# yardenas/ethz-safe-learning

Hardware: NVIDIA B200
Metric: CEM-MPC plans/sec (PointGoal1 shape; ensemble transitions/sec alongside) (higher is better)
Workload: dtype bf16

## Files before the change

### ethz-safe-learning_b200/csrc/rollout_tc.cu

```cuda
#include <cuda_bf16.h>

#include <cstdlib>
#include <type_traits>

#include "common.cuh"
#include "internal.h"
#include "rollout_params.cuh"
#include "tc_head.cuh"
#include "tc_ptx.cuh"

namespace simba {

#ifdef SIMBA_TC_TIMELINE
#define TL(ev)                                                                                   \
  do {                                                                                           \
    if (tl_who >= 0 && blockIdx.x == 0)                                                          \
      prm.timeline[(tl_who * 64 + tl_t) * 64 + (ev)] = clock64();  \
  } while (0)
#else
#define TL(ev) do { } while (0)
#endif

namespace {

constexpr int kU = 128;
constexpr int kMaxO = 60;
constexpr int kAtomBytes = 128 * 128;
constexpr int kBiasBlockBytes = 4096;
constexpr int kBoundThreads = 640;

__host__ __device__ constexpr uint32_t tc_weight_bytes(int L) { return kAtomBytes + (uint32_t)L * 2 * kAtomBytes; }
__host__ __device__ constexpr uint32_t tc_member_bytes(int L) {
  return tc_weight_bytes(L) + (uint32_t)(L + 1) * kBiasBlockBytes;
}
__host__ __device__ constexpr bool tc_l0_pad_bias(int in_dim) { return in_dim + 2 <= 64; }

struct TileInfo {
  int32_t member, k0, count, valid;
};

template <int NB, int kThreads>
struct NoiseSmem {
  uint4* base;
  __device__ __forceinline__ uint4 get4(int b) const { return base[b * kThreads]; }
  __device__ __forceinline__ void put4(int b, uint4 v) { base[b * kThreads] = v; }
  __device__ __forceinline__ void put4_dyn(int b, uint4 v) { base[b * kThreads] = v; }
};
template <int NB>
struct NoiseRegs {
  uint4 v[NB];
  __device__ __forceinline__ uint4 get4(int b) const { return v[b]; }
  __device__ __forceinline__ void put4(int b, uint4 x) { v[b] = x; }
  __device__ __forceinline__ void put4_dyn(int b, uint4 x) {
#pragma unroll
    for (int i = 0; i < NB; ++i)
      if (i == b) v[i] = x;
  }
};

struct AStoreTmem {
  uint32_t t_a;
  __device__ __forceinline__ void store8(int k0, uint32_t p0, uint32_t p1, uint32_t p2, uint32_t p3) const {
    const uint32_t pk[4] = {p0, p1, p2, p3};
    tmem_st<4>(t_a + (uint32_t)(k0 >> 1), pk);
  }
};

struct AStorePair {
  uint32_t t_a;
  uint32_t peer_slot;
  uint32_t buf_off;
  uint32_t peer_bar;
  __device__ __forceinline__ void store8(int k0, uint32_t p0, uint32_t p1, uint32_t p2, uint32_t p3) const {
    const uint32_t pk[4] = {p0, p1, p2, p3};
    tmem_st<4>(t_a + (uint32_t)(k0 >> 1), pk);
    st_async_v4(peer_slot + buf_off, p0, p1, p2, p3, peer_bar);
  }
};

}

template <int NTILES, int Q, bool PAIR, bool TRAJ, bool FWD = false>
__device__ __forceinline__ void rollout_tc_body(const RolloutParams& prm) {
  static_assert(!PAIR || (NTILES == 1 && Q == 4), "the pair variant is the one-tile latency configuration");
  static_assert(!(PAIR && TRAJ), "the trajectory form has no pair variant");
  static_assert(!FWD || TRAJ, "the forward form is a trajectory form");
  constexpr int kTileThreads = Q * 128;
  constexpr int kTileWarps = Q * 4;
  constexpr int kEpiThreads = NTILES * kTileThreads;
  constexpr int kEpiWarps = kEpiThreads / 32;
  constexpr int OW = (PAIR ? 32 : 64) / Q;
  constexpr int NSL = PAIR ? 2 * Q : Q;
  constexpr int NB = OW / 8;
  constexpr int HCOLS = 128 / Q;
  constexpr bool kDbl = NTILES == 1;
  static_assert(!kDbl || Q == 4, "the one-tile variants split the columns into halves of two column groups");
  constexpr int kTmemCols = 512;
  constexpr uint32_t kStateCol = kDbl ? 256 : NTILES * 128;
  constexpr uint32_t kACol = kDbl ? 320 : NTILES * 192;
  constexpr bool kPark = NTILES > 1;
  constexpr int kBarAcc = 2, kBarA = 2 + NTILES, kBarPart = 2 + 2 * NTILES, kBarFree = 2 + 3 * NTILES;
  constexpr int kBarAccHi = 6, kBarAHi = 7;
  extern __shared__ __align__(1024) uint8_t smem_raw[];
  const RowGeom& g = prm.g;
  const int L = prm.L;
  const int H = g.H;
  const int O = g.O, A = g.A;
  const int warp = threadIdx.x >> 5, lane = threadIdx.x & 31;
  const uint32_t crank = PAIR ? cluster_ctarank() : 0u;
  const int n_items = (prm.n_tiles + NTILES - 1) / NTILES;
  const int cta_item0 = PAIR ? (int)(blockIdx.x >> 1) : (int)blockIdx.x;
  const int n_ctas = PAIR ? (int)(gridDim.x >> 1) : (int)gridDim.x;
  const bool l0_pad_bias = tc_l0_pad_bias(O + A);
  constexpr int n_quarters = 4;
  constexpr int tile_bar_threads = Q * 128 + 32;
  constexpr int half_bar_threads = Q * 64 + 32;

  const uint32_t w_bytes = tc_weight_bytes(L);
  uint8_t* w_smem = smem_raw;
  uint8_t* biask_smem = w_smem + w_bytes;
  uint8_t* ones_smem = biask_smem + (L + 1) * 4096;
  float* scale_smem = reinterpret_cast<float*>(ones_smem + 4096);
  float* pen_smem = scale_smem + 128;
  const int nparts = TRAJ ? 1 : 1 + prm.scorer.n_constraints;
  float* part_smem = pen_smem + kHeadParts * 64;
  const int part_buf_floats = NTILES * NSL * nparts * 128;
  uint4* xch_smem = reinterpret_cast<uint4*>(part_smem + (PAIR ? 2 : 1) * part_buf_floats);
  uint4* noise_smem = xch_smem + (PAIR ? 2 * Q * 128 : 0);
  uint32_t* rs_smem = reinterpret_cast<uint32_t*>(noise_smem + (kPark ? NB * kEpiThreads : 0));
  uint64_t* bars = reinterpret_cast<uint64_t*>(rs_smem + NTILES * 8 * 128);
  uint32_t* tmem_slot = reinterpret_cast<uint32_t*>(bars + 1 + NTILES + 2 + (kDbl ? 1 : 0));
  TileInfo* tinfo = reinterpret_cast<TileInfo*>(tmem_slot + 2);
  uint64_t* seed_sh = reinterpret_cast<uint64_t*>(tinfo + NTILES);
  int32_t* w_state_sh = reinterpret_cast<int32_t*>(seed_sh + 1);

  const uint32_t bar_w = smem_u32(&bars[0]);

#ifdef SIMBA_TC_TIMELINE
#define TLK(k) do { if (blockIdx.x == 0 && threadIdx.x == 0) { prm.timeline[(3 * 64) * 64 + (k)] = clock64(); \
    unsigned long long gt_; asm volatile("mov.u64 %0, %%globaltimer;" : "=l"(gt_)); \
    prm.timeline[(3 * 64 + 10 + prm.iteration) * 64 + (k)] = (long long)gt_; } } while (0)
#else
#define TLK(k) do { } while (0)
#endif
  TLK(0);
  pdl_launch_dependents();
  auto item_member = [&](int item) {
    int wm = -1;
    for (int q = 0; q < NTILES; ++q)
      if (item * NTILES + q < prm.n_tiles && prm.tiles[item * NTILES + q].count > 0) wm = prm.tiles[item * NTILES + q].member;
    return wm;
  };
  auto stage_weights = [&](int wm) {
    const uint8_t* wsrc = reinterpret_cast<const uint8_t*>(prm.w_tc) + (size_t)wm * prm.w_tc_member_bytes;
    const uint32_t bk_bytes = (uint32_t)(L + 1) * 4096u;
    mbar_expect_tx(bar_w, w_bytes + bk_bytes);
    uint32_t off = 0;
    for (int l = 0; l <= L; ++l) {
      const uint32_t nb = (l == 0) ? kAtomBytes : 2 * kAtomBytes;
      bulk_g2s(smem_u32(w_smem + off), wsrc + off, nb, bar_w);
      off += nb;
    }
    bulk_g2s(smem_u32(biask_smem), wsrc + (prm.w_tc_member_bytes - bk_bytes), bk_bytes, bar_w);
    w_state_sh[0] = wm;
    w_state_sh[1] += 1;
  };
  if (threadIdx.x == 0) {
    mbar_init(bar_w, 1);
#pragma unroll
    for (int j = 0; j < NTILES; ++j) {
      mbar_init(smem_u32(&bars[1 + j]), 1);
    }
    if (kDbl) mbar_init(smem_u32(&bars[3 + NTILES]), 1);
    if (PAIR) {
      mbar_init(smem_u32(&bars[1 + NTILES]), 1);
      mbar_init(smem_u32(&bars[2 + NTILES]), 1);
    }
    fence_barrier_init();
    w_state_sh[0] = -1;
    w_state_sh[1] = 0;
    const int wm = cta_item0 < n_items ? item_member(cta_item0) : -1;
    if (wm >= 0) stage_weights(wm);
  }
  auto load_tile = [&](int ti) {
    TileInfo info{0, 0, 0, 0};
    if (ti < prm.n_tiles) {
      const Tile t = prm.tiles[ti];
      info.member = t.member; info.k0 = t.k0; info.count = t.count;
      info.valid = t.count > 0 ? 1 : 0;
    }
    return info;
  };
  if (threadIdx.x < NTILES) tinfo[threadIdx.x] = load_tile(cta_item0 * NTILES + threadIdx.x);
  if (warp == 0) tmem_alloc(smem_u32(tmem_slot), kTmemCols);
  if (warp < kEpiWarps) {
    for (int i = threadIdx.x; i < 1024; i += kEpiThreads) {
      const int byte = i * 4;
      const bool first = ((byte & 255) < 128) && ((byte & 15) == 0);
      reinterpret_cast<uint32_t*>(ones_smem)[i] = first ? 0x3F803F80u : 0u;
    }
    fence_proxy_async();
    if constexpr (TRAJ) {
      head_tables_init(scale_smem, pen_smem, prm.tc_scale_a, prm.tc_scale_b, simba_scorer_t{},
                       l0_pad_bias ? O + A : -1, threadIdx.x, kEpiThreads);
    } else {
      head_tables_init(scale_smem, pen_smem, prm.tc_scale_a, prm.tc_scale_b, prm.scorer,
                       l0_pad_bias ? O + A : -1, threadIdx.x, kEpiThreads);
    }
  }
  if (PAIR && threadIdx.x == 0) {
    const uint32_t per_step = crank == 0 ? (uint32_t)(kEpiThreads * 4 * nparts) : 0u;
    mbar_expect_tx(smem_u32(&bars[2 + NTILES]), per_step + (uint32_t)(kEpiThreads * 16));
    const uint32_t b0 = per_step + (1 < H ? (uint32_t)(kEpiThreads * 16) : 0u);
    if (b0 != 0u) mbar_expect_tx(smem_u32(&bars[1 + NTILES]), b0);
  }
  tc_fence_before();
  __syncthreads();
  if (PAIR) cluster_sync_all();
  tc_fence_after();
  const uint32_t tmem_base = *tmem_slot;
  TLK(1);
  constexpr bool kLateWait = PAIR;
  if (!kLateWait) pdl_wait_prior_grid();
  TLK(2);
  if (threadIdx.x == 0) *seed_sh = prm.seed_ptr ? *prm.seed_ptr : prm.seed;
  auto tile_active = [&](const TileInfo& t) {
    if (prm.active == nullptr) return true;
    const int m = g.rows_per_state[t.member];
    bool any = false;
    for (int s = t.k0 / m; s <= (t.k0 + t.count - 1) / m; ++s) any = any || prm.active[s] != 0;
    return any;
  };
  auto late_gate = [&](const TileInfo& t) {
    if (!kLateWait) return true;
    pdl_wait_prior_grid();
    return tile_active(t);
  };
  uint32_t ph = 0;

#pragma unroll 1
  for (int item = cta_item0; item < n_items; item += n_ctas) {
  if (threadIdx.x < NTILES) {
    TileInfo info = tinfo[threadIdx.x];
    if (item != cta_item0) info = load_tile(item * NTILES + threadIdx.x);
    if (!kLateWait && info.valid) info.valid = tile_active(info) ? 1 : 0;
    tinfo[threadIdx.x] = info;
  }
  __syncthreads();
  bool any_valid = false;
  int member = -1;
#pragma unroll
  for (int j = 0; j < NTILES; ++j)
    if (tinfo[j].valid) { any_valid = true; member = tinfo[j].member; }
  if (threadIdx.x == 0 && any_valid && member != w_state_sh[0]) {
    if (w_state_sh[1] > 0) mbar_wait(bar_w, (uint32_t)(w_state_sh[1] - 1) & 1u);
    stage_weights(member);
  }
  __syncthreads();

  if (any_valid) {
    if (kDbl && warp == kEpiWarps + 2 * NTILES) {
      if (tinfo[0].valid && late_gate(tinfo[0])) {
        const uint32_t bar_lo = smem_u32(&bars[1]), bar_hi = smem_u32(&bars[3 + NTILES]);
        for (int t = 0; t < H; ++t) {
          for (int layer = 0; layer <= L; ++layer) {
            mbar_wait(layer < L ? bar_lo : bar_hi, ph);
            tc_fence_before();
            named_bar_arrive_n(kBarAcc, half_bar_threads);
            mbar_wait(bar_hi, ph);
            ph ^= 1;
            tc_fence_before();
            named_bar_arrive_n(kBarAccHi, half_bar_threads);
          }
        }
      }
    } else if (warp >= kEpiWarps + NTILES) {
      const int j = warp - kEpiWarps - NTILES;
      const TileInfo tis = tinfo[j];
      auto xbytes = [&](int t) -> uint32_t {
        return (crank == 0 ? (uint32_t)(kEpiThreads * 4 * nparts) : 0u) + (t + 1 < H ? (uint32_t)(kEpiThreads * 16) : 0u);
      };
      const uint32_t xbar = smem_u32(&bars[1 + NTILES]);
      if (PAIR && tis.valid && crank != 0 && late_gate(tis)) {
        for (int ts = -1; ts + 1 < H; ++ts) {
          mbar_wait(xbar + 8u * ((uint32_t)ts & 1u), (uint32_t)((ts + 1) >> 1) & 1u);
          if (lane == 0 && xbytes(ts + 2) != 0u) mbar_expect_tx(xbar + 8u * ((uint32_t)ts & 1u), xbytes(ts + 2));
        }
      }
      if (!TRAJ && tis.valid && crank == 0) {
        const simba_scorer_t& sc = prm.scorer;
        const bool done_first = objective_done_first(prm.objective);
        uint32_t* my_rs = rs_smem + j * 8 * 128 + lane;
        const float* part_tile0 = part_smem + (j * NSL * nparts) * 128;
#pragma unroll 1
        for (int i = 0; i < n_quarters; ++i) {
          const int row = lane + 32 * i;
#pragma unroll
          for (int f = 0; f < 7; ++f) my_rs[f * 128 + 32 * i] = 0u;
          my_rs[7 * 128 + 32 * i] = row < tis.count ? (uint32_t)decode_row(g, tis.member, tis.k0 + row).out : 0xffffffffu;
        }
        const bool live = late_gate(tis);
        for (int ts = -1; live && ts < H; ++ts) {
          named_bar_sync_n(kBarPart + j, tile_bar_threads);
          const float* part_tile = part_tile0;
          if (PAIR) {
            mbar_wait(xbar + 8u * ((uint32_t)ts & 1u), (uint32_t)((ts + 1) >> 1) & 1u);
            if (lane == 0 && ts + 2 < H) mbar_expect_tx(xbar + 8u * ((uint32_t)ts & 1u), xbytes(ts + 2));
            part_tile += (ts & 1) * part_buf_floats;
          }
#pragma unroll 1
          for (int i = 0; i < n_quarters; ++i) {
            uint32_t* q = my_rs + 32 * i;
            float nd, nc;
            head_combine<NSL>(sc, part_tile + lane + 32 * i, nparts, nd, nc);
            if (ts < 0) {
              q[4 * 128] = __float_as_uint(nd);
              q[5 * 128] = __float_as_uint(nc);
            } else {
              RowScore rs;
              rs.cum = __uint_as_float(q[0]);
              rs.costsum = __uint_as_float(q[128]);
              rs.cmask = (uint64_t)q[2 * 128] | ((uint64_t)q[3 * 128] << 32);
              rs.dist = __uint_as_float(q[4 * 128]);
              rs.cost = __uint_as_float(q[5 * 128]);
              rs.done = q[6 * 128] != 0u;
              head_score_step(rs, sc, done_first, ts, nd, nc);
              q[0] = __float_as_uint(rs.cum);
              q[128] = __float_as_uint(rs.costsum);
              q[2 * 128] = (uint32_t)rs.cmask;
              q[3 * 128] = (uint32_t)(rs.cmask >> 32);
              q[4 * 128] = __float_as_uint(rs.dist);
              q[5 * 128] = __float_as_uint(rs.cost);
              q[6 * 128] = rs.done ? 1u : 0u;
            }
          }
          if (ts + 1 < H) named_bar_arrive_n(kBarFree + j, tile_bar_threads);
        }
        if (live && prm.row_return != nullptr) {
#pragma unroll 1
          for (int i = 0; i < n_quarters; ++i) {
            const uint32_t* q = my_rs + 32 * i;
            const uint32_t slot = q[7 * 128];
            if (slot != 0xffffffffu) {
              prm.row_return[slot] = __uint_as_float(q[0]);
              prm.row_costmask[slot] = (uint64_t)q[2 * 128] | ((uint64_t)q[3 * 128] << 32);
              prm.row_costsum[slot] = __uint_as_float(q[128]);
            }
          }
        }
      }
    } else if (warp >= kEpiWarps) {
      const int j = warp - kEpiWarps;
      if (tinfo[j].valid) {
        const uint32_t bar_acc = smem_u32(&bars[1 + j]);
        const uint32_t d_tmem = tmem_base + (uint32_t)j * 128;
        const uint32_t a_tmem = tmem_base + (uint32_t)(kACol + j * 64);
        const uint64_t ones_desc = umma_desc_k16_noswizzle(smem_u32(ones_smem));
        mbar_wait(bar_w, (uint32_t)(w_state_sh[1] - 1) & 1u);
#ifdef SIMBA_TC_TIMELINE
        const int tl_who = (j == 0 && lane == 0) ? 2 : -1;
#endif
        const bool live = late_gate(tinfo[j]);
        if constexpr (kDbl) {
          const uint32_t bar_acc_hi = smem_u32(&bars[3 + NTILES]);
          constexpr uint32_t kIdesc64 = umma_idesc_n(64u), kIdesc32 = umma_idesc_n(32u);
          uint32_t par = 0;
          auto mma4 = [&](uint32_t d, uint32_t a, uint64_t b, uint32_t idesc, int kb) {
#pragma unroll
            for (int k = 0; k < 4; ++k)
              umma_bf16_ts(d, a + (uint32_t)(kb + k) * 8, b + (uint64_t)(((kb ? kAtomBytes : 0) + k * 32) >> 4), idesc,
                           (kb + k) > 0 ? 1u : 0u);
          };
          auto mma_bias = [&](uint32_t d, uint32_t bias_sm, uint32_t col, uint32_t idesc) {
            umma_bf16(d, ones_desc, umma_desc_k16_noswizzle(bias_sm + col * 32), idesc, 1u);
          };
          for (int t = 0; live && t < H; ++t) {
#ifdef SIMBA_TC_TIMELINE
            const int tl_t = t;
#endif
            {
              const uint32_t d = d_tmem + par * 128, a = a_tmem + par * 64;
              const uint64_t b = umma_desc_sw128(smem_u32(w_smem));
              const uint32_t bias_sm = smem_u32(biask_smem);
              named_bar_sync_n(kBarA, half_bar_threads);
              named_bar_sync_n(kBarAHi, half_bar_threads);
              tc_fence_after();
              TL(0);
              if (elect_one()) {
                mma4(d, a, b, kIdesc64, 0);
                if (!l0_pad_bias) mma_bias(d, bias_sm, 0u, kIdesc64);
                umma_commit(bar_acc);
                mma4(d + 64, a, b + (uint64_t)((64 * 128) >> 4), kIdesc64, 0);
                if (!l0_pad_bias) mma_bias(d + 64, bias_sm, 64u, kIdesc64);
                umma_commit(bar_acc_hi);
              }
              TL(1);
              __syncwarp();
              par ^= 1;
            }
            for (int layer = 1; layer <= L; ++layer) {
              const uint32_t d = d_tmem + par * 128, a = a_tmem + par * 64;
              const bool own_head = PAIR && layer == L;
              const uint32_t c0 = own_head ? crank * 32 : 0u, c1 = own_head ? 64u + crank * 32 : 64u;
              const uint32_t idesc = own_head ? kIdesc32 : kIdesc64;
              const uint64_t bw = umma_desc_sw128(smem_u32(w_smem + kAtomBytes + (layer - 1) * 2 * kAtomBytes));
              const uint64_t b0 = bw + (uint64_t)((c0 * 128) >> 4), b1 = bw + (uint64_t)((c1 * 128) >> 4);
              const uint32_t bias_sm = smem_u32(biask_smem + layer * 4096);
              named_bar_sync_n(kBarA, half_bar_threads);
              tc_fence_after();
              TL(2 * layer);
              if (elect_one()) {
                mma4(d + c0, a, b0, idesc, 0);
                mma4(d + c1, a, b1, idesc, 0);
              }
              TL(2 * layer + 1);
              __syncwarp();
              named_bar_sync_n(kBarAHi, half_bar_threads);
              tc_fence_after();
              TL(20 + 2 * layer);
              if (elect_one()) {
                mma4(d + c0, a, b0, idesc, 4);
                mma_bias(d + c0, bias_sm, c0, idesc);
                umma_commit(bar_acc);
                mma4(d + c1, a, b1, idesc, 4);
                mma_bias(d + c1, bias_sm, c1, idesc);
                umma_commit(bar_acc_hi);
              }
              TL(21 + 2 * layer);
              __syncwarp();
              par ^= 1;
            }
          }
        } else
        for (int t = 0; live && t < H; ++t) {
#ifdef SIMBA_TC_TIMELINE
          const int tl_t = t;
#endif
          for (int layer = 0; layer <= L; ++layer) {
            named_bar_sync_n(kBarA + j, tile_bar_threads);
            tc_fence_after();
            TL(2 * layer);
            if (elect_one()) {
              const uint32_t woff = (layer == 0) ? 0u : (uint32_t)(kAtomBytes + (layer - 1) * 2 * kAtomBytes);
              const uint64_t b0 = umma_desc_sw128(smem_u32(w_smem + woff));
#pragma unroll
              for (int k = 0; k < 4; ++k)
                umma_bf16_ts(d_tmem, a_tmem + (uint32_t)k * 8, b0 + (uint64_t)((k * 32) >> 4), kIdesc, k > 0 ? 1u : 0u);
              if (layer > 0) {
#pragma unroll
                for (int k = 4; k < 8; ++k)
                  umma_bf16_ts(d_tmem, a_tmem + (uint32_t)k * 8, b0 + (uint64_t)((kAtomBytes + (k - 4) * 32) >> 4),
                               kIdesc, 1u);
              }
              if (layer > 0 || !l0_pad_bias)
                umma_bf16(d_tmem, ones_desc, umma_desc_k16_noswizzle(smem_u32(biask_smem + layer * 4096)), kIdesc, 1u);
              umma_commit(bar_acc);
            }
            TL(2 * layer + 1);
            __syncwarp();
            mbar_wait(bar_acc, ph);
            ph ^= 1;
            tc_fence_before();
            named_bar_arrive_n(kBarAcc + j, tile_bar_threads);
          }
        }
      }
    } else {
      const int j = warp / kTileWarps;
      const int wl = warp - j * kTileWarps;
      const int cgp = wl >> 2;
      const int r = (wl & 3) * 32 + lane;
      const TileInfo ti = tinfo[j];
      if (ti.valid) {
        const bool row_ok = r < ti.count;
        const RowId id = decode_row(g, ti.member, ti.k0 + (row_ok ? r : 0));
        const uint32_t lane_base = tmem_base + ((uint32_t)((wl & 3) * 32) << 16);
        const uint32_t t_acc = lane_base + (uint32_t)j * 128;
        const uint32_t t_a = lane_base + (uint32_t)(kACol + j * 64);
        const float* act_ptr = prm.actions + ((int64_t)id.s * g.N + id.i_global) * prm.action_stride;
        const simba_scorer_t& sc = prm.scorer;

        HeadCtx hc;
        hc.t_acc = t_acc;
        hc.t_state = lane_base + (uint32_t)(kStateCol + j * 64);
        hc.o_base = (PAIR ? (int)crank * 32 : 0) + cgp * OW;
        hc.O = O; hc.A = A;
        hc.slice_bits = TRAJ ? 0u : head_slice_bits<OW>(sc, hc.o_base);
        hc.n_constraints = TRAJ ? 0 : sc.n_constraints;
        hc.scale_smem = scale_smem;
        hc.pen_smem = pen_smem;
        float* part_slot0 = part_smem + ((j * NSL + (int)crank * Q + cgp) * nparts) * 128 + r;
        hc.part = part_slot0 + (PAIR ? part_buf_floats : 0);
        typename std::conditional<PAIR, AStorePair, AStoreTmem>::type astore;
        astore.t_a = t_a;
        const uint32_t my_xbar = smem_u32(&bars[1 + NTILES]);
        const uint32_t peer_xbar = PAIR ? cluster_map_u32(my_xbar, crank ^ 1u) : 0u;
        const bool keeps_score = !TRAJ && (!PAIR || crank == 0);
        const uint32_t part_remote0 = (PAIR && crank != 0) ? cluster_map_u32(smem_u32(part_slot0), 0u) : 0u;
        if constexpr (PAIR) {
          astore.peer_slot = cluster_map_u32(smem_u32(xch_smem + cgp * 128 + r), crank ^ 1u);
          astore.buf_off = (uint32_t)(Q * 128 * sizeof(uint4));
          astore.peer_bar = peer_xbar + 8u;
          if (crank != 0) {
            hc.part_remote = part_remote0 + (uint32_t)(part_buf_floats * sizeof(float));
            hc.part_mbar = peer_xbar + 8u;
          }
        }
        auto exchange = [&](int t, bool next_step) {
          if constexpr (PAIR) {
            const uint32_t b = (uint32_t)t & 1u;
            if (next_step) {
              mbar_wait(my_xbar + 8u * b, (uint32_t)((t + 1) >> 1) & 1u);
              const uint4 v = xch_smem[(b * Q + cgp) * 128 + r];
              const uint32_t pk[4] = {v.x, v.y, v.z, v.w};
              tmem_st<4>(astore.t_a + (uint32_t)((((int)crank ^ 1) * 32 + cgp * 8) >> 1), pk);
            }
          }
        };
        const float* s0_ptr = prm.states + (prm.state_per_row ? id.r_global : (int64_t)id.s) * prm.state_stride;
        typename std::conditional<FWD, ForwardSink, typename std::conditional<TRAJ, TrajSink, NoTraj>::type>::type sink{};
        if constexpr (FWD) {
          sink = ForwardSink{prm.mu_out, prm.var_out, prm.sample_out, row_ok ? (int)id.out : -1, O};
        } else if constexpr (TRAJ) {
          sink.row = row_ok ? prm.traj_out + id.out * (int64_t)(H + 1) * O : nullptr;
          sink.O = O;
        }

#ifdef SIMBA_TC_TIMELINE
        const int tl_who = (j == 0 && lane == 0) ? (wl == 0 ? 0 : (wl == kTileWarps - 1 ? 1 : -1)) : -1;
        int tl_t = 0;
#endif
        static_assert(!kDbl || kBarAccHi - kBarAcc == kBarAHi - kBarA, "one offset selects both barriers of a half");
        const int bar_off = kDbl ? (cgp >= Q / 2 ? kBarAHi - kBarA : 0) : j;
        const int bar_acc_mine = kBarAcc + bar_off, bar_a_mine = kBarA + bar_off;
        const int hand_off_threads = kDbl ? half_bar_threads : tile_bar_threads;
        auto publish_a = [&]() {
          tmem_st_wait();
          tc_fence_before();
          named_bar_arrive_n(bar_a_mine, hand_off_threads);
        };
        auto wait_accumulator = [&]() {
          named_bar_sync_n(bar_acc_mine, hand_off_threads);
          tc_fence_after();
        };
        auto gemm_par = [&](int t, int l) { return (uint32_t)(t * (L + 1) + l) & 1u; };

        const bool owns_actions = TRAJ ? (O < hc.o_base + OW) && (O + A > hc.o_base)
                                       : (O >= hc.o_base) && (O < hc.o_base + OW);
        float act_pf[4] = {0.f, 0.f, 0.f, 0.f};
        auto prefetch_actions = [&](int tn) {
          if (owns_actions && row_ok && tn < H) {
#pragma unroll
            for (int a = 0; a < 4; ++a)
              if (a < A) act_pf[a] = act_ptr[tn * A + a];
          }
        };

        typename std::conditional<kPark, NoiseSmem<NB, kEpiThreads>, NoiseRegs<NB>>::type noise;
        if constexpr (kPark) noise.base = noise_smem + threadIdx.x;
#pragma unroll
        for (int b = 0; b < NB; ++b) noise.put4(b, make_uint4(0u, 0u, 0u, 0u));
        const uint32_t c3_noise = (uint32_t)id.s | (kStreamNoise << 28);
        const uint32_t row32 = (uint32_t)id.r_global;
        const float* eps_row = prm.eps == nullptr ? nullptr
            : prm.eps + ((int64_t)id.s * H * ((int64_t)g.P * g.N) + id.r_global) * O;
        const int64_t eps_step = (int64_t)g.P * g.N * O;
        const uint64_t seed64 = *seed_sh;
        const uint2 key = make_uint2((uint32_t)seed64, (uint32_t)(seed64 >> 32));
        const uint32_t c2_base = (uint32_t)prm.iteration << 16;
        auto make_noise = [&](int b, int t) {
          const int o0 = hc.o_base + b * 8;
          if (o0 >= O) return;
          uint4 z;
          if (FWD || eps_row != nullptr) {
            z = external_noise8_bf16(eps_row + t * eps_step, o0, O);
          } else {
#ifdef SIMBA_TC_TIMELINE
            {
              PhiloxState p{(uint32_t)(o0 >> 3), row32, (uint32_t)t | c2_base, c3_noise, key.x, key.y};
              TL(50);
              philox_rounds<10>(p);
              if (p.c0 == 0x12345u) TL(53);
              TL(51);
              z = philox_finish_noise8_bf16(p);
              if (z.x == 0x12345u) TL(53);
              TL(52);
            }
#else
            z = philox_noise8_bf16(key, (uint32_t)(o0 >> 3), row32, (uint32_t)t | c2_base, c3_noise);
#endif
            if (o0 + 8 > O) z = mask_noise8(z, o0, O);
          }
          noise.put4_dyn(b, z);
        };
        float s0v[8];
        if constexpr (PAIR) {
#pragma unroll
          for (int i = 0; i < 8; ++i) s0v[i] = (row_ok && hc.o_base + i < O) ? s0_ptr[hc.o_base + i] : 0.0f;
        }
        const bool live = late_gate(ti);
        if (live) {
        prefetch_actions(0);
        if constexpr (PAIR) head_first_pass_vals(hc, astore, s0v, act_pf);
        else head_first_pass<OW>(hc, astore, s0_ptr, row_ok, act_pf, sink);
        prefetch_actions(1);
        exchange(-1, true);
        publish_a();
        TLK(3);
        if (keeps_score) named_bar_arrive_n(kBarPart + j, tile_bar_threads);

        PhiloxState ps{0u, 0u, 0u, 0u, 0u, 0u};
        for (int t = 0; t < H; ++t) {
#ifdef SIMBA_TC_TIMELINE
          tl_t = t;
#endif
          TL(0);
          if (owns_actions) {
            if constexpr (TRAJ) head_store_own_actions<OW>(hc, act_pf);
            else head_store_actions(hc, act_pf);
          }
          prefetch_actions(t + 2);
          for (int l = 0; l < L; ++l) {
            wait_accumulator();
            TL(1 + l * 4);
            {
              constexpr int NLD = HCOLS / 32;
              uint32_t v[NLD][32];
#pragma unroll
              for (int i = 0; i < NLD; ++i) tmem_ld<32>(t_acc + (kDbl ? gemm_par(t, l) * 128 : 0u) + (uint32_t)(cgp * HCOLS + i * 32), v[i]);
              tmem_ld_wait();
#pragma unroll
              for (int i = 0; i < NLD; ++i) {
                uint32_t pk[16];
#pragma unroll
                for (int q = 0; q < 16; ++q)
                  pk[q] = pack_relu_bf16(__uint_as_float(v[i][2 * q]), __uint_as_float(v[i][2 * q + 1]));
                tmem_st<16>(t_a + (kDbl ? (gemm_par(t, l) ^ 1u) * 64 : 0u) + (uint32_t)((cgp * HCOLS + i * 32) / 2), pk);
              }
            }
            TL(2 + l * 4);
            publish_a();
            TL(3 + l * 4);
            if (prm.sampling_propagation) {
              if (!FWD && NTILES == 1 && L >= 2 * NB && eps_row == nullptr) {
                const int b = l >> 1, o0 = hc.o_base + b * 8;
                if (b < NB && o0 < O) {
                  if ((l & 1) == 0) {
                    ps = PhiloxState{(uint32_t)(o0 >> 3), row32, (uint32_t)t | c2_base, c3_noise, key.x, key.y};
                    philox_rounds<10>(ps);
                  } else {
                    uint4 z = philox_finish_noise8_bf16(ps);
                    if (o0 + 8 > O) z = mask_noise8(z, o0, O);
                    noise.put4_dyn(b, z);
                  }
                }
              } else {
                if (l < NB) make_noise(l, t);
                if (l == L - 1)
                  for (int b = L; b < NB; ++b) make_noise(b, t);
              }
            }
            TL(4 + l * 4);
          }

          wait_accumulator();
          if (keeps_score) named_bar_sync_n(kBarFree + j, tile_bar_threads);
          TL(40);
          if constexpr (PAIR) {
            hc.part = part_slot0 + (t & 1) * part_buf_floats;
            astore.buf_off = (uint32_t)((t & 1) * Q * 128 * sizeof(uint4));
            astore.peer_bar = peer_xbar + 8u * ((uint32_t)t & 1u);
            if (crank != 0) {
              hc.part_remote = part_remote0 + (uint32_t)((t & 1) * part_buf_floats * sizeof(float));
              hc.part_mbar = astore.peer_bar;
            }
          }
          if constexpr (TRAJ && !FWD) {
            if (sink.row != nullptr) sink.row += O;
          }
          if constexpr (kDbl) {
            hc.t_acc = t_acc + gemm_par(t, L) * 128;
            astore.t_a = t_a + (gemm_par(t, L) ^ 1u) * 64;
          }
          if constexpr (FWD) head_step_pass<OW, true>(hc, noise, astore, false, sink);
          else if (prm.sampling_propagation) head_step_pass<OW, true>(hc, noise, astore, t + 1 < H, sink);
          else head_step_pass<OW, false>(hc, noise, astore, t + 1 < H, sink);
          TL(41);
          exchange(t, t + 1 < H);
          if (t + 1 < H) publish_a();
          if (keeps_score) named_bar_arrive_n(kBarPart + j, tile_bar_threads);
          TL(42);
        }
        TLK(6);
        }
      }
    }
  }

  tc_fence_before();
  __syncthreads();
  tc_fence_after();
  }

  if (threadIdx.x == 0 && w_state_sh[1] > 0) mbar_wait(bar_w, (uint32_t)(w_state_sh[1] - 1) & 1u);
  tc_fence_before();
  __syncthreads();
  TLK(4);
  if (warp == 0) tmem_dealloc(tmem_base, kTmemCols);
  TLK(5);
}

template <int NTILES, int Q, bool PAIR>
__global__ void __launch_bounds__(kBoundThreads, 1) rollout_tc_kernel(const RolloutParams prm) {
  rollout_tc_body<NTILES, Q, PAIR, false>(prm);
}

template <int NTILES, int Q>
__global__ void __launch_bounds__(kBoundThreads, 1) unfold_tc_kernel(const RolloutParams prm) {
  rollout_tc_body<NTILES, Q, false, true>(prm);
}

template <int NTILES, int Q>
__global__ void __launch_bounds__(kBoundThreads, 1) forward_tc_kernel(const RolloutParams prm) {
  rollout_tc_body<NTILES, Q, false, true, true>(prm);
}

static size_t tc_smem_bytes(int L, int ntiles, int q, int nparts, bool pair = false) {
  size_t b = tc_member_bytes(L) + 4096;
  b += 128 * sizeof(float);
  b += kHeadParts * 64 * sizeof(float);
  b += (size_t)ntiles * q * nparts * 128 * sizeof(float) * (pair ? 4 : 1);
  if (pair) b += (size_t)2 * q * 128 * sizeof(uint4);
  if (ntiles > 1)
    b += (size_t)(64 / q / 8) * (ntiles * q * 128) * sizeof(uint4);
  b += (size_t)8 * ntiles * 128 * sizeof(uint32_t);
  b += (3 + ntiles + (ntiles == 1 ? 1 : 0)) * sizeof(uint64_t) + 2 * sizeof(uint32_t) + ntiles * sizeof(TileInfo) + sizeof(uint64_t) + 2 * sizeof(int32_t);
  return b + 1024;
}

constexpr size_t kMaxSmem = 227 * 1024;

bool rollout_tc_supported(int O, int A, int L, int U) {
  return U >= 1 && U <= kU && O >= 1 && O <= kMaxO && O + A <= 64 && A <= 4 && L >= 1 &&
         tc_smem_bytes(L, 1, 4, kHeadParts) + 1024 <= kMaxSmem;
}

int64_t rollout_tc_pack(const ModelWeights& mw, std::vector<uint16_t>& img) {
  const auto& c = mw.cfg;
  const int L = c.n_layers, E = c.ensemble_size, U = c.units, O = c.obs_dim, IN = c.obs_dim + c.act_dim;
  const int64_t member_bytes = tc_member_bytes(L);
  img.assign((size_t)E * member_bytes / 2, 0);
  for (int e = 0; e < E; ++e) {
    uint16_t* w = &img[(size_t)e * member_bytes / 2];
    uint16_t* bias_k16 = w + tc_weight_bytes(L) / 2;
    for (int l = 0; l <= L; ++l) {
      const int K = l == 0 ? IN : U;
      auto weight = [&](int k, int n) -> uint16_t {
        if (l == 0 && tc_l0_pad_bias(IN) && (k == IN || k == IN + 1) && n < U) {
          uint16_t hi, lo;
          bf16_split(mw.bias(e, 0)[n], hi, lo);
          return k == IN ? hi : lo;
        }
        if (k >= K) return 0;
        if (l < L) return n < U ? bf16_bits(mw.kernel(e, l)[(size_t)k * U + n]) : 0;
        if (n < O) return bf16_bits(mw.kernel(e, L)[(size_t)k * O + n]);
        if (n >= 64 && n < 64 + O) return bf16_bits(kLog2e * mw.kernel(e, L + 1)[(size_t)k * O + (n - 64)]);
        return 0;
      };
      const int atoms = l == 0 ? 1 : 2;
      for (int at = 0; at < atoms; ++at)
        for (int n = 0; n < 128; ++n)
          for (int kk = 0; kk < 64; ++kk) w[(at * kAtomBytes + sw128_offset(n, kk)) / 2] = weight(at * 64 + kk, n);
      w += atoms * kAtomBytes / 2;
      for (int n = 0; n < 128; ++n) {
        float bv = 0.0f;
        if (l < L) bv = n < U ? mw.bias(e, l)[n] : 0.0f;
        else if (n < O) bv = mw.bias(e, L)[n];
        else if (n >= 64 && n < 64 + O) bv = kLog2e * mw.bias(e, L + 1)[n - 64];
        uint16_t* bk = bias_k16 + l * kBiasBlockBytes / 2 + (n / 8) * 128 + (n % 8) * 8;
        bf16_split(bv, bk[0], bk[1]);
      }
    }
  }
  return member_bytes;
}

bool rollout_tc_two_tiles_fit(int L, int n_constraints) {
  return tc_smem_bytes(L, 2, 2, 1 + n_constraints) + 1024 <= kMaxSmem;
}

bool rollout_tc_pair_fits(int L, int n_constraints) {
  return tc_smem_bytes(L, 1, 4, 1 + n_constraints, true) + 1024 <= kMaxSmem;
}

template <int NTILES, int Q, bool PAIR, bool TRAJ, bool FWD = false>
static cudaError_t launch_variant(const RolloutParams& prm, cudaStream_t stream) {
  void (*kern)(const RolloutParams) = rollout_tc_kernel<NTILES, Q, PAIR>;
  if constexpr (FWD) kern = forward_tc_kernel<NTILES, Q>;
  else if constexpr (TRAJ) kern = unfold_tc_kernel<NTILES, Q>;
  const size_t smem = tc_smem_bytes(prm.L, NTILES, Q, TRAJ ? 1 : 1 + prm.scorer.n_constraints, PAIR);
  const int n_items = (prm.n_tiles + NTILES - 1) / NTILES;
  const int sms = prm.n_sms;
  if (sms <= 0) return cudaErrorInvalidValue;
  const int grid = PAIR ? 2 * n_items : (n_items < sms ? n_items : sms);
  return launch_kernel(kern, grid, NTILES * Q * 128 + 64 * NTILES + (NTILES == 1 ? 32 : 0), smem, stream, PAIR ? 2 : 1, prm.pdl, prm);
}

cudaError_t launch_rollout_tc(const RolloutParams& prm, cudaStream_t stream) {
  if (prm.mu_out != nullptr) {
    switch (prm.kernel) {
      case RolloutKernel::kTcOneCta: return launch_variant<1, 4, false, true, true>(prm, stream);
      case RolloutKernel::kTcTwoTile: return launch_variant<2, 2, false, true, true>(prm, stream);
      default: return cudaErrorInvalidValue;
    }
  }
  if (prm.traj_out == nullptr) {
    switch (prm.kernel) {
      case RolloutKernel::kTcOneCta: return launch_variant<1, 4, false, false>(prm, stream);
      case RolloutKernel::kTcPair: return launch_variant<1, 4, true, false>(prm, stream);
      case RolloutKernel::kTcTwoTile: return launch_variant<2, 2, false, false>(prm, stream);
      default: return cudaErrorInvalidValue;
    }
  }
  switch (prm.kernel) {
    case RolloutKernel::kTcOneCta: return launch_variant<1, 4, false, true>(prm, stream);
    case RolloutKernel::kTcTwoTile: return launch_variant<2, 2, false, true>(prm, stream);
    default: return cudaErrorInvalidValue;
  }
}

}
```

### ethz-safe-learning_b200/csrc/tc_head.cuh

```cuda
#pragma once
#include "common.cuh"
#include "tc_ptx.cuh"

namespace simba {
namespace {

constexpr int kHeadParts = 1 + SIMBA_MAX_CONSTRAINTS;

__device__ __forceinline__ uint32_t box_muller_pair_bf16(uint32_t w) {
  const float fa = __uint_as_float(__byte_perm(w, 0x4b000000u, 0x7610));
  const float fb = __uint_as_float(__byte_perm(w, 0x4b000000u, 0x7632));
  const float ua = fmaf(fa, 1.52587890625e-05f, -128.0f + 7.62939453125e-06f);
  const float ub = fmaf(fb, 1.52587890625e-05f, -128.0f + 7.62939453125e-06f);
  float lg, r, sn, cs;
  const float th = 6.283185307179586f * ub;
  asm("lg2.approx.ftz.f32 %0, %1;" : "=f"(lg) : "f"(ua));
  asm("sqrt.approx.ftz.f32 %0, %1;" : "=f"(r) : "f"(-1.3862943611198906f * lg));
  asm("sin.approx.ftz.f32 %0, %1;" : "=f"(sn) : "f"(th));
  asm("cos.approx.ftz.f32 %0, %1;" : "=f"(cs) : "f"(th));
  return pack_bf16(r * cs, r * sn);
}

struct PhiloxState {
  uint32_t c0, c1, c2, c3, k0, k1;
};
template <int kRounds>
__device__ __forceinline__ void philox_rounds(PhiloxState& p) {
#pragma unroll
  for (int r = 0; r < kRounds; ++r) {
    uint32_t lo0, hi0, lo1, hi1;
    asm("{\n\t.reg .b64 p;\n\tmul.wide.u32 p, %2, %3;\n\tmov.b64 {%0, %1}, p;\n\t}" : "=r"(lo0), "=r"(hi0) : "r"(p.c0), "r"(kPhiloxM0));
    asm("{\n\t.reg .b64 p;\n\tmul.wide.u32 p, %2, %3;\n\tmov.b64 {%0, %1}, p;\n\t}" : "=r"(lo1), "=r"(hi1) : "r"(p.c2), "r"(kPhiloxM1));
    const uint32_t n0 = hi1 ^ p.c1 ^ p.k0, n2 = hi0 ^ p.c3 ^ p.k1;
    p.c1 = lo1; p.c3 = lo0; p.c0 = n0; p.c2 = n2;
    p.k0 += kPhiloxW0; p.k1 += kPhiloxW1;
  }
}
__device__ __forceinline__ uint4 philox_finish_noise8_bf16(const PhiloxState& p) {
  return make_uint4(box_muller_pair_bf16(p.c0), box_muller_pair_bf16(p.c1), box_muller_pair_bf16(p.c2),
                    box_muller_pair_bf16(p.c3));
}
__device__ __forceinline__ uint4 philox_noise8_bf16(uint2 key, uint32_t c0, uint32_t c1, uint32_t c2,
                                                    uint32_t c3) {
  PhiloxState p{c0, c1, c2, c3, key.x, key.y};
  philox_rounds<10>(p);
  return philox_finish_noise8_bf16(p);
}

__device__ __forceinline__ uint4 mask_noise8(uint4 z, int o0, int O) {
  uint32_t w[4] = {z.x, z.y, z.z, z.w};
#pragma unroll
  for (int i = 0; i < 4; ++i) {
    if (o0 + 2 * i >= O) w[i] = 0u;
    else if (o0 + 2 * i + 1 >= O) w[i] &= 0xffffu;
  }
  return make_uint4(w[0], w[1], w[2], w[3]);
}

__device__ __forceinline__ uint4 external_noise8_bf16(const float* ep, int o0, int O) {
  float z[8];
#pragma unroll
  for (int q = 0; q < 8; ++q) z[q] = (o0 + q < O) ? ep[o0 + q] : 0.0f;
  return make_uint4(pack_bf16(z[0], z[1]), pack_bf16(z[2], z[3]), pack_bf16(z[4], z[5]), pack_bf16(z[6], z[7]));
}

template <int kTW = 64>
__device__ __forceinline__ void head_tables_init(float* scale_smem, float* pen_smem, const float* sa,
                                                 const float* sb, const simba_scorer_t& sc, int ones_at,
                                                 int tid, int nthreads) {
  for (int i = tid; i < kTW; i += nthreads) {
    const bool one = ones_at >= 0 && (i == ones_at || i == ones_at + 1);
    scale_smem[i] = one ? 0.0f : sa[i];
    scale_smem[kTW + i] = one ? 1.0f : sb[i];
    const bool in_goal = sc.goal_dist_index >= 0 ? (i == sc.goal_dist_index) : (i >= sc.goal_begin && i < sc.goal_end);
    pen_smem[i] = in_goal ? 0.0f : INFINITY;
    for (int q = 0; q < SIMBA_MAX_CONSTRAINTS; ++q)
      pen_smem[(1 + q) * kTW + i] =
          (q < sc.n_constraints && i >= sc.con_begin[q] && i < sc.con_end[q]) ? 0.0f : INFINITY;
  }
}

template <int OW>
__device__ __forceinline__ uint32_t head_slice_bits(const simba_scorer_t& sc, int o_base) {
  uint32_t bits = 0;
#pragma unroll
  for (int c = 0; c < OW / 8; ++c) {
    const int lo = o_base + c * 8, hi = lo + 8;
    if (sc.goal_dist_index >= 0 ? (sc.goal_dist_index >= lo && sc.goal_dist_index < hi)
                                : (sc.goal_begin < hi && sc.goal_end > lo)) bits |= 1u << (c * 5);
    for (int q = 0; q < sc.n_constraints; ++q)
      if (sc.con_begin[q] < hi && sc.con_end[q] > lo) bits |= 1u << (c * 5 + 1 + q);
  }
  return bits;
}

struct HeadCtx {
  uint32_t t_acc;
  uint32_t t_state;
  int o_base;
  int O, A;
  uint32_t slice_bits;
  int n_constraints;
  const float* scale_smem;
  const float* pen_smem;
  float* part;
  uint32_t part_remote = 0, part_mbar = 0;
};

__device__ __forceinline__ float head_stddev(float x_log2e) {
  float e, l, sd;
  asm("ex2.approx.ftz.f32 %0, %1;" : "=f"(e) : "f"(fminf(x_log2e, 120.0f)));
  asm("lg2.approx.ftz.f32 %0, %1;" : "=f"(l) : "f"(1.0f + e));
  asm("sqrt.approx.ftz.f32 %0, %1;" : "=f"(sd) : "f"(fmaf(l, 0.6931471805599453f, 1e-4f)));
  return sd;
}

__device__ __forceinline__ float slice_min8(const float (&v)[8], const float* pen, float acc) {
  const float4 p0 = *reinterpret_cast<const float4*>(pen);
  const float4 p1 = *reinterpret_cast<const float4*>(pen + 4);
  const float a = fminf(fminf(v[0] + p0.x, v[1] + p0.y), fminf(v[2] + p0.z, v[3] + p0.w));
  const float b = fminf(fminf(v[4] + p1.x, v[5] + p1.y), fminf(v[6] + p1.z, v[7] + p1.w));
  return fminf(acc, fminf(a, b));
}

template <int kTW, class AStore>
__device__ __forceinline__ void head_chunk_tail(const HeadCtx& c, const AStore& astore, int oc, uint32_t bits,
                                                const float (&sv)[8], bool write_next, float& gmin,
                                                float (&cmin)[SIMBA_MAX_CONSTRAINTS]) {
  if (bits) {
    if (bits & 1u) gmin = slice_min8(sv, c.pen_smem + oc, gmin);
    if (bits >> 1) {
#pragma unroll
      for (int q = 0; q < SIMBA_MAX_CONSTRAINTS; ++q)
        if ((bits >> (1 + q)) & 1u) cmin[q] = slice_min8(sv, c.pen_smem + (1 + q) * kTW + oc, cmin[q]);
    }
  }
  if (write_next) {
    const ulonglong2 a0 = *reinterpret_cast<const ulonglong2*>(c.scale_smem + oc);
    const ulonglong2 a1 = *reinterpret_cast<const ulonglong2*>(c.scale_smem + oc + 4);
    const ulonglong2 b0 = *reinterpret_cast<const ulonglong2*>(c.scale_smem + kTW + oc);
    const ulonglong2 b1 = *reinterpret_cast<const ulonglong2*>(c.scale_smem + kTW + oc + 4);
    float x[8];
    f2_unpack(f2_fma(f2_pack(sv[0], sv[1]), a0.x, b0.x), x[0], x[1]);
    f2_unpack(f2_fma(f2_pack(sv[2], sv[3]), a0.y, b0.y), x[2], x[3]);
    f2_unpack(f2_fma(f2_pack(sv[4], sv[5]), a1.x, b1.x), x[4], x[5]);
    f2_unpack(f2_fma(f2_pack(sv[6], sv[7]), a1.y, b1.y), x[6], x[7]);
    astore.store8(oc, pack_bf16(x[0], x[1]), pack_bf16(x[2], x[3]), pack_bf16(x[4], x[5]), pack_bf16(x[6], x[7]));
  }
}

__device__ __forceinline__ void head_store_actions(const HeadCtx& c, const float (&act)[4]) {
  const uint32_t v[4] = {__float_as_uint(act[0]), __float_as_uint(act[1]), __float_as_uint(act[2]),
                         __float_as_uint(act[3])};
  tmem_st<4>(c.t_state + c.O, v);
}

__device__ __forceinline__ void head_publish(const HeadCtx& c, float gmin, const float (&cmin)[SIMBA_MAX_CONSTRAINTS]) {
  if (c.part_remote != 0u) {
    st_async_b32(c.part_remote, __float_as_uint(gmin), c.part_mbar);
#pragma unroll
    for (int q = 0; q < SIMBA_MAX_CONSTRAINTS; ++q)
      if (q < c.n_constraints) st_async_b32(c.part_remote + (uint32_t)((1 + q) * 128 * 4), __float_as_uint(cmin[q]), c.part_mbar);
    return;
  }
  c.part[0] = gmin;
#pragma unroll
  for (int q = 0; q < SIMBA_MAX_CONSTRAINTS; ++q)
    if (q < c.n_constraints) c.part[(1 + q) * 128] = cmin[q];
}

struct NoTraj {
  static constexpr bool kScore = true, kState = true;
  __device__ __forceinline__ void put8(int, const float (&)[8]) const {}
};
struct TrajSink {
  static constexpr bool kScore = false, kState = true;
  float* row;
  int O;
  __device__ __forceinline__ void put8(int oc, const float (&v)[8]) const {
    if (row == nullptr || oc >= O) return;
    float* p = row + oc;
    if (oc + 8 <= O && (reinterpret_cast<uintptr_t>(p) & 15u) == 0) {
      __stcs(reinterpret_cast<float4*>(p), make_float4(v[0], v[1], v[2], v[3]));
      __stcs(reinterpret_cast<float4*>(p + 4), make_float4(v[4], v[5], v[6], v[7]));
    } else if (oc + 8 <= O && (reinterpret_cast<uintptr_t>(p) & 7u) == 0) {
#pragma unroll
      for (int i = 0; i < 8; i += 2) __stcs(reinterpret_cast<float2*>(p + i), make_float2(v[i], v[i + 1]));
    } else {
#pragma unroll
      for (int i = 0; i < 8; ++i)
        if (oc + i < O) __stcs(p + i, v[i]);
    }
  }
};
struct ForwardSink {
  static constexpr bool kScore = false, kState = false;
  float* mu;
  float* var;
  float* sample;
  int row;
  int O;
  __device__ __forceinline__ void head8(int oc, const uint32_t (&mu_bits)[8], const float (&v)[8],
                                        const float (&smp)[8]) const {
    if (row < 0) return;
    const int64_t off = (int64_t)row * O;
    float m[8];
#pragma unroll
    for (int i = 0; i < 8; ++i) m[i] = __uint_as_float(mu_bits[i]);
    TrajSink{mu + off, O}.put8(oc, m);
    TrajSink{var + off, O}.put8(oc, v);
    if (sample != nullptr) TrajSink{sample + off, O}.put8(oc, smp);
  }
  __device__ __forceinline__ void put8(int, const float (&)[8]) const {}
};

template <int OW>
__device__ __forceinline__ void head_store_own_actions(const HeadCtx& c, const float (&act)[4]) {
#pragma unroll
  for (int a = 0; a < 4; ++a) {
    if (a < c.A && c.O + a >= c.o_base && c.O + a < c.o_base + OW) {
      const uint32_t v[1] = {__float_as_uint(act[a])};
      tmem_st<1>(c.t_state + (uint32_t)(c.O + a), v);
    }
  }
}

template <int OW, int kTW = 64, class AStore, class Sink = NoTraj>
__device__ __forceinline__ void head_first_pass(const HeadCtx& c, const AStore& astore, const float* s0_ptr,
                                                bool row_ok, const float (&act0)[4], const Sink& sink = Sink()) {
  float gmin = INFINITY, cmin[SIMBA_MAX_CONSTRAINTS];
#pragma unroll
  for (int q = 0; q < SIMBA_MAX_CONSTRAINTS; ++q) cmin[q] = INFINITY;
#pragma unroll 1
  for (int ch = 0; ch < OW / 8; ++ch) {
    const int oc = c.o_base + ch * 8;
    float sv[8];
    uint32_t st[8];
#pragma unroll
    for (int i = 0; i < 8; ++i) {
      sv[i] = (row_ok && oc + i < c.O) ? s0_ptr[oc + i] : 0.0f;
#pragma unroll
      for (int a = 0; a < 4; ++a)
        if (oc + i == c.O + a) sv[i] = act0[a];
      st[i] = __float_as_uint(sv[i]);
    }
    tmem_st<8>(c.t_state + oc, st);
    sink.put8(oc, sv);
    head_chunk_tail<kTW>(c, astore, oc, Sink::kScore ? (c.slice_bits >> (ch * 5)) & 31u : 0u, sv, true, gmin, cmin);
  }
  if constexpr (Sink::kScore) head_publish(c, gmin, cmin);
}

template <class AStore>
__device__ __forceinline__ void head_first_pass_vals(const HeadCtx& c, const AStore& astore, const float (&s0v)[8],
                                                     const float (&act0)[4]) {
  float gmin = INFINITY, cmin[SIMBA_MAX_CONSTRAINTS];
#pragma unroll
  for (int q = 0; q < SIMBA_MAX_CONSTRAINTS; ++q) cmin[q] = INFINITY;
  const int oc = c.o_base;
  float sv[8];
  uint32_t st[8];
#pragma unroll
  for (int i = 0; i < 8; ++i) {
    sv[i] = s0v[i];
#pragma unroll
    for (int a = 0; a < 4; ++a)
      if (oc + i == c.O + a) sv[i] = act0[a];
    st[i] = __float_as_uint(sv[i]);
  }
  tmem_st<8>(c.t_state + oc, st);
  head_chunk_tail<64>(c, astore, oc, c.slice_bits & 31u, sv, true, gmin, cmin);
  head_publish(c, gmin, cmin);
}

template <int OW, bool kSample, int kVar = 64, int kTW = 64, class Noise, class AStore, class Sink = NoTraj>
__device__ __forceinline__ void head_step_pass(const HeadCtx& c, const Noise& noise, const AStore& astore,
                                               bool write_next, const Sink& sink = Sink()) {
  constexpr int NCH = OW / 8;
  float gmin = INFINITY, cmin[SIMBA_MAX_CONSTRAINTS];
#pragma unroll
  for (int q = 0; q < SIMBA_MAX_CONSTRAINTS; ++q) cmin[q] = INFINITY;
  static_assert(Sink::kState || kSample, "the forward form forms the variance");
  uint32_t vm[2][8], vv[2][8], st[2][8];
  tmem_ld<8>(c.t_acc + c.o_base, vm[0]);
  if (kSample) tmem_ld<8>(c.t_acc + kVar + c.o_base, vv[0]);
  if constexpr (Sink::kState) tmem_ld<8>(c.t_state + c.o_base, st[0]);
#pragma unroll
  for (int ch = 0; ch < NCH; ++ch) {
    const int oc = c.o_base + ch * 8;
    const int cur = ch & 1, nxt = cur ^ 1;
    tmem_ld_wait();
    if (ch + 1 < NCH) {
      tmem_ld<8>(c.t_acc + oc + 8, vm[nxt]);
      if (kSample) tmem_ld<8>(c.t_acc + kVar + oc + 8, vv[nxt]);
      if constexpr (Sink::kState) tmem_ld<8>(c.t_state + oc + 8, st[nxt]);
    }
    float sv[8];
    if (kSample) {
      const uint4 nz = noise.get4(ch);
      const uint32_t nw[4] = {nz.x, nz.y, nz.z, nz.w};
      const f32x2 kOne = f2_pack(1.0f, 1.0f);
      const f32x2 kLn2 = f2_pack(0.6931471805599453f, 0.6931471805599453f), kFloor = f2_pack(1e-4f, 1e-4f);
      float hv[8], hd[8];
#pragma unroll
      for (int q = 0; q < 8; q += 2) {
        float e0, e1, l0, l1, s0, s1;
        asm("ex2.approx.ftz.f32 %0, %1;" : "=f"(e0) : "f"(fminf(__uint_as_float(vv[cur][q]), 120.0f)));
        asm("ex2.approx.ftz.f32 %0, %1;" : "=f"(e1) : "f"(fminf(__uint_as_float(vv[cur][q + 1]), 120.0f)));
        f2_unpack(f2_add(f2_pack(e0, e1), kOne), l0, l1);
        asm("lg2.approx.ftz.f32 %0, %1;" : "=f"(l0) : "f"(l0));
        asm("lg2.approx.ftz.f32 %0, %1;" : "=f"(l1) : "f"(l1));
        f2_unpack(f2_fma(f2_pack(l0, l1), kLn2, kFloor), s0, s1);
        if constexpr (!Sink::kState) { hv[q] = s0; hv[q + 1] = s1; }
        asm("sqrt.approx.ftz.f32 %0, %1;" : "=f"(s0) : "f"(s0));
        asm("sqrt.approx.ftz.f32 %0, %1;" : "=f"(s1) : "f"(s1));
        const f32x2 eps = f2_pack(__uint_as_float(nw[q >> 1] << 16), __uint_as_float(nw[q >> 1] & 0xffff0000u));
        const f32x2 mu = f2_pack(__uint_as_float(vm[cur][q]), __uint_as_float(vm[cur][q + 1]));
        if constexpr (Sink::kState) {
          const f32x2 old = f2_pack(__uint_as_float(st[cur][q]), __uint_as_float(st[cur][q + 1]));
          f2_unpack(f2_add(old, f2_fma(f2_pack(s0, s1), eps, mu)), sv[q], sv[q + 1]);
        } else {
          f2_unpack(f2_fma(f2_pack(s0, s1), eps, mu), hd[q], hd[q + 1]);
        }
      }
      if constexpr (!Sink::kState) sink.head8(oc, vm[cur], hv, hd);
    } else {
#pragma unroll
      for (int q = 0; q < 8; ++q) sv[q] = __uint_as_float(st[cur][q]) + __uint_as_float(vm[cur][q]);
    }
    if constexpr (Sink::kState) {
      {
        uint32_t so[8];
#pragma unroll
        for (int i = 0; i < 8; ++i) so[i] = __float_as_uint(sv[i]);
        tmem_st<8>(c.t_state + oc, so);
      }
      sink.put8(oc, sv);
      head_chunk_tail<kTW>(c, astore, oc, Sink::kScore ? (c.slice_bits >> (ch * 5)) & 31u : 0u, sv, write_next,
                           gmin, cmin);
    }
  }
  if constexpr (Sink::kScore) head_publish(c, gmin, cmin);
}

__device__ __forceinline__ float closest_from_min(float m, float D) {
  const float w = __fsub_rn(D, __fmul_rn(D, __fsub_rn(1.0f, m)));
  return fminf(fmaxf(w, 0.0f), D);
}

template <int Q>
__device__ __forceinline__ void head_combine(const simba_scorer_t& sc, const float* part_row, int nparts,
                                             float& dist, float& cost) {
  float g = INFINITY;
#pragma unroll
  for (int c = 0; c < Q; ++c) g = fminf(g, part_row[(c * nparts) * 128]);
  dist = sc.goal_dist_index >= 0 ? fmaxf(g, 0.0f) : closest_from_min(g, sc.lidar_max_dist);
  float cst = 0.0f;
  for (int q = 0; q < sc.n_constraints; ++q) {
    float m = INFINITY;
#pragma unroll
    for (int c = 0; c < Q; ++c) m = fminf(m, part_row[(c * nparts + 1 + q) * 128]);
    cst += (closest_from_min(m, sc.lidar_max_dist) <= sc.con_size[q]) ? 1.0f : 0.0f;
  }
  cost = sc.constrain_indicator ? (cst > 0.0f ? 1.0f : 0.0f) : cst;
}

__device__ __forceinline__ void head_score_step(RowScore& rs, const simba_scorer_t& sc, bool done_first, int t,
                                                float next_dist, float next_cost) {
  const bool goal = rs.dist <= sc.goal_threshold;
  const float rew = step_reward(sc, rs.dist, next_dist, goal);
  if (done_first) {
    rs.done = rs.done || goal;
    if (!rs.done && rs.cost > 0.0f) rs.cmask |= (1ull << t);
    rs.cum += rs.done ? 0.0f : rew;
  } else {
    rs.cum += rs.done ? 0.0f : rew;
    if (!rs.done && rs.cost > 0.0f) rs.cmask |= (1ull << t);
    rs.done = rs.done || goal;
  }
  rs.costsum += rs.cost;
  rs.dist = next_dist;
  rs.cost = next_cost;
}

}
}
```

### ethz-safe-learning_b200/csrc/tc_ptx.cuh

```cuda
#pragma once
#include <cuda_bf16.h>

#include <cstdint>

namespace simba {
namespace {

__device__ __forceinline__ uint32_t smem_u32(const void* p) {
  return (uint32_t)__cvta_generic_to_shared(p);
}
__device__ __forceinline__ void mbar_init(uint32_t bar, uint32_t count) {
  asm volatile("mbarrier.init.shared::cta.b64 [%0], %1;" ::"r"(bar), "r"(count));
}
__device__ __forceinline__ void mbar_arrive(uint32_t bar) {
  asm volatile("mbarrier.arrive.shared::cta.b64 _, [%0];" ::"r"(bar) : "memory");
}
__device__ __forceinline__ void mbar_expect_tx(uint32_t bar, uint32_t bytes) {
  asm volatile("mbarrier.arrive.expect_tx.shared::cta.b64 _, [%0], %1;" ::"r"(bar), "r"(bytes)
               : "memory");
}
constexpr uint32_t kSuspendHintNs = 100000;
__device__ __forceinline__ bool mbar_try_wait(uint32_t bar, uint32_t parity) {
  uint32_t ok;
  asm volatile(
      "{\n\t.reg .pred p;\n\t"
#ifdef SIMBA_TC_SPIN
      "mbarrier.try_wait.parity.shared::cta.b64 p, [%1], %2;\n\t"
#else
      "mbarrier.try_wait.parity.shared::cta.b64 p, [%1], %2, %3;\n\t"
#endif
      "selp.u32 %0, 1, 0, p;\n\t}"
      : "=r"(ok)
      : "r"(bar), "r"(parity), "r"(kSuspendHintNs)
      : "memory");
  return ok != 0;
}
__device__ __forceinline__ void mbar_wait(uint32_t bar, uint32_t parity) {
  uint32_t spins = 0;
  while (!mbar_try_wait(bar, parity)) {
    if (++spins > (1u << 20)) __trap();
  }
}
__device__ __forceinline__ void fence_barrier_init() {
  asm volatile("fence.mbarrier_init.release.cluster;" ::: "memory");
}
__device__ __forceinline__ void fence_proxy_async() {
  asm volatile("fence.proxy.async.shared::cta;" ::: "memory");
}
__device__ __forceinline__ void tc_fence_before() {
  asm volatile("tcgen05.fence::before_thread_sync;" ::: "memory");
}
__device__ __forceinline__ void tc_fence_after() {
  asm volatile("tcgen05.fence::after_thread_sync;" ::: "memory");
}
__device__ __forceinline__ void bulk_g2s(uint32_t dst, const void* src, uint32_t bytes, uint32_t bar) {
  asm volatile(
      "cp.async.bulk.shared::cluster.global.mbarrier::complete_tx::bytes [%0], [%1], %2, [%3];" ::"r"(dst),
      "l"(src), "r"(bytes), "r"(bar)
      : "memory");
}
__device__ __forceinline__ void tmem_alloc(uint32_t dst_smem, uint32_t ncols) {
  asm volatile("tcgen05.alloc.cta_group::1.sync.aligned.shared::cta.b32 [%0], %1;" ::"r"(dst_smem),
               "r"(ncols)
               : "memory");
  asm volatile("tcgen05.relinquish_alloc_permit.cta_group::1.sync.aligned;" ::: "memory");
}
__device__ __forceinline__ void tmem_dealloc(uint32_t taddr, uint32_t ncols) {
  asm volatile("tcgen05.dealloc.cta_group::1.sync.aligned.b32 %0, %1;" ::"r"(taddr), "r"(ncols)
               : "memory");
}
__device__ __forceinline__ void umma_bf16(uint32_t d_tmem, uint64_t a_desc, uint64_t b_desc,
                                          uint32_t idesc, uint32_t accumulate) {
  asm volatile(
      "{\n\t.reg .pred p;\n\t"
      "setp.ne.b32 p, %4, 0;\n\t"
      "tcgen05.mma.cta_group::1.kind::f16 [%0], %1, %2, %3, p;\n\t}" ::"r"(d_tmem),
      "l"(a_desc), "l"(b_desc), "r"(idesc), "r"(accumulate)
      : "memory");
}
__device__ __forceinline__ void umma_bf16_ts(uint32_t d_tmem, uint32_t a_tmem, uint64_t b_desc,
                                             uint32_t idesc, uint32_t accumulate) {
  asm volatile(
      "{\n\t.reg .pred p;\n\t"
      "setp.ne.b32 p, %4, 0;\n\t"
      "tcgen05.mma.cta_group::1.kind::f16 [%0], [%1], %2, %3, p;\n\t}" ::"r"(d_tmem),
      "r"(a_tmem), "l"(b_desc), "r"(idesc), "r"(accumulate)
      : "memory");
}
__device__ __forceinline__ void umma_commit(uint32_t bar) {
  asm volatile("tcgen05.commit.cta_group::1.mbarrier::arrive::one.shared::cluster.b64 [%0];" ::"r"(bar)
               : "memory");
}
template <int N>
__device__ __forceinline__ void tmem_ld(uint32_t taddr, uint32_t (&v)[N]) {
  static_assert(N == 4 || N == 8 || N == 16 || N == 32, "unsupported TMEM load width");
  if constexpr (N == 4)
    asm volatile("tcgen05.ld.sync.aligned.32x32b.x4.b32 {%0, %1, %2, %3}, [%4];"
                 : "=r"(v[0]), "=r"(v[1]), "=r"(v[2]), "=r"(v[3]) : "r"(taddr) : "memory");
  if constexpr (N == 8)
    asm volatile("tcgen05.ld.sync.aligned.32x32b.x8.b32 {%0, %1, %2, %3, %4, %5, %6, %7}, [%8];"
                 : "=r"(v[0]), "=r"(v[1]), "=r"(v[2]), "=r"(v[3]), "=r"(v[4]), "=r"(v[5]), "=r"(v[6]), "=r"(v[7]) : "r"(taddr) : "memory");
  if constexpr (N == 16)
    asm volatile("tcgen05.ld.sync.aligned.32x32b.x16.b32 {%0, %1, %2, %3, %4, %5, %6, %7, %8, %9, %10, %11, %12, %13, %14, %15}, [%16];"
                 : "=r"(v[0]), "=r"(v[1]), "=r"(v[2]), "=r"(v[3]), "=r"(v[4]), "=r"(v[5]), "=r"(v[6]), "=r"(v[7]), "=r"(v[8]), "=r"(v[9]), "=r"(v[10]), "=r"(v[11]), "=r"(v[12]), "=r"(v[13]), "=r"(v[14]), "=r"(v[15]) : "r"(taddr) : "memory");
  if constexpr (N == 32)
    asm volatile("tcgen05.ld.sync.aligned.32x32b.x32.b32 {%0, %1, %2, %3, %4, %5, %6, %7, %8, %9, %10, %11, %12, %13, %14, %15, %16, %17, %18, %19, %20, %21, %22, %23, %24, %25, %26, %27, %28, %29, %30, %31}, [%32];"
                 : "=r"(v[0]), "=r"(v[1]), "=r"(v[2]), "=r"(v[3]), "=r"(v[4]), "=r"(v[5]), "=r"(v[6]), "=r"(v[7]), "=r"(v[8]), "=r"(v[9]), "=r"(v[10]), "=r"(v[11]), "=r"(v[12]), "=r"(v[13]), "=r"(v[14]), "=r"(v[15]), "=r"(v[16]), "=r"(v[17]), "=r"(v[18]), "=r"(v[19]), "=r"(v[20]), "=r"(v[21]), "=r"(v[22]), "=r"(v[23]), "=r"(v[24]), "=r"(v[25]), "=r"(v[26]), "=r"(v[27]), "=r"(v[28]), "=r"(v[29]), "=r"(v[30]), "=r"(v[31]) : "r"(taddr) : "memory");
}
template <int N>
__device__ __forceinline__ void tmem_st(uint32_t taddr, const uint32_t (&v)[N]) {
  static_assert(N == 1 || N == 4 || N == 8 || N == 16, "unsupported TMEM store width");
  if constexpr (N == 1)
    asm volatile("tcgen05.st.sync.aligned.32x32b.x1.b32 [%0], {%1};" :: "r"(taddr), "r"(v[0]) : "memory");
  if constexpr (N == 4)
    asm volatile("tcgen05.st.sync.aligned.32x32b.x4.b32 [%0], {%1, %2, %3, %4};"
                 :: "r"(taddr), "r"(v[0]), "r"(v[1]), "r"(v[2]), "r"(v[3]) : "memory");
  if constexpr (N == 8)
    asm volatile("tcgen05.st.sync.aligned.32x32b.x8.b32 [%0], {%1, %2, %3, %4, %5, %6, %7, %8};"
                 :: "r"(taddr), "r"(v[0]), "r"(v[1]), "r"(v[2]), "r"(v[3]), "r"(v[4]), "r"(v[5]), "r"(v[6]), "r"(v[7]) : "memory");
  if constexpr (N == 16)
    asm volatile("tcgen05.st.sync.aligned.32x32b.x16.b32 [%0], {%1, %2, %3, %4, %5, %6, %7, %8, %9, %10, %11, %12, %13, %14, %15, %16};"
                 :: "r"(taddr), "r"(v[0]), "r"(v[1]), "r"(v[2]), "r"(v[3]), "r"(v[4]), "r"(v[5]), "r"(v[6]), "r"(v[7]), "r"(v[8]), "r"(v[9]), "r"(v[10]), "r"(v[11]), "r"(v[12]), "r"(v[13]), "r"(v[14]), "r"(v[15]) : "memory");
}
__device__ __forceinline__ void tmem_ld_wait() {
  asm volatile("tcgen05.wait::ld.sync.aligned;" ::: "memory");
}
__device__ __forceinline__ void tmem_st_wait() {
  asm volatile("tcgen05.wait::st.sync.aligned;" ::: "memory");
}
__device__ __forceinline__ uint32_t pack_relu_bf16(float a, float b) {
  uint32_t r;
  asm("cvt.rn.relu.bf16x2.f32 %0, %1, %2;" : "=r"(r) : "f"(b), "f"(a));
  return r;
}
__device__ __forceinline__ uint32_t pack_bf16(float a, float b) {
  uint32_t r;
  asm("cvt.rn.bf16x2.f32 %0, %1, %2;" : "=r"(r) : "f"(b), "f"(a));
  return r;
}
__device__ __forceinline__ float2 add2(uint32_t lo, uint32_t hi, float2 b) {
  unsigned long long a = ((unsigned long long)hi << 32) | lo, bb, r;
  bb = ((unsigned long long)__float_as_uint(b.y) << 32) | __float_as_uint(b.x);
  asm("add.rn.f32x2 %0, %1, %2;" : "=l"(r) : "l"(a), "l"(bb));
  return make_float2(__uint_as_float((uint32_t)r), __uint_as_float((uint32_t)(r >> 32)));
}
typedef unsigned long long f32x2;
__device__ __forceinline__ f32x2 f2_pack(float lo, float hi) {
  f32x2 r;
  asm("mov.b64 %0, {%1, %2};" : "=l"(r) : "f"(lo), "f"(hi));
  return r;
}
__device__ __forceinline__ void f2_unpack(f32x2 v, float& lo, float& hi) {
  asm("mov.b64 {%0, %1}, %2;" : "=f"(lo), "=f"(hi) : "l"(v));
}
__device__ __forceinline__ f32x2 f2_fma(f32x2 a, f32x2 b, f32x2 c) {
  f32x2 r;
  asm("fma.rn.f32x2 %0, %1, %2, %3;" : "=l"(r) : "l"(a), "l"(b), "l"(c));
  return r;
}
__device__ __forceinline__ f32x2 f2_mul(f32x2 a, f32x2 b) {
  f32x2 r;
  asm("mul.rn.f32x2 %0, %1, %2;" : "=l"(r) : "l"(a), "l"(b));
  return r;
}
__device__ __forceinline__ f32x2 f2_add(f32x2 a, f32x2 b) {
  f32x2 r;
  asm("add.rn.f32x2 %0, %1, %2;" : "=l"(r) : "l"(a), "l"(b));
  return r;
}

__device__ __forceinline__ void st_shared_v4(uint32_t addr, uint32_t a, uint32_t b, uint32_t c,
                                             uint32_t d) {
  asm volatile("st.shared.v4.b32 [%0], {%1, %2, %3, %4};" ::"r"(addr), "r"(a), "r"(b), "r"(c), "r"(d)
               : "memory");
}
__device__ __forceinline__ void pdl_launch_dependents() {
  asm volatile("griddepcontrol.launch_dependents;" ::: "memory");
}
__device__ __forceinline__ void pdl_wait_prior_grid() {
  asm volatile("griddepcontrol.wait;" ::: "memory");
}
__device__ __forceinline__ float sqrt_approx(float x) {
  float r;
  asm("sqrt.approx.ftz.f32 %0, %1;" : "=f"(r) : "f"(x));
  return r;
}
template <int kThreads>
__device__ __forceinline__ void named_bar_sync(int id) {
  asm volatile("bar.sync %0, %1;" ::"r"(id), "n"(kThreads) : "memory");
}

__device__ __forceinline__ bool elect_one() {
  uint32_t pred;
  asm volatile(
      "{\n\t.reg .pred p;\n\t"
      "elect.sync _|p, 0xffffffff;\n\t"
      "selp.u32 %0, 1, 0, p;\n\t}"
      : "=r"(pred));
  return pred != 0;
}

template <int kThreads>
__device__ __forceinline__ void named_bar_arrive(int id) {
  asm volatile("bar.arrive %0, %1;" ::"r"(id), "n"(kThreads) : "memory");
}

__device__ __forceinline__ void named_bar_sync_n(int id, int threads) {
  asm volatile("bar.sync %0, %1;" ::"r"(id), "r"(threads) : "memory");
}
__device__ __forceinline__ void named_bar_arrive_n(int id, int threads) {
  asm volatile("bar.arrive %0, %1;" ::"r"(id), "r"(threads) : "memory");
}

__device__ __forceinline__ uint32_t cluster_ctarank() {
  uint32_t r;
  asm volatile("mov.u32 %0, %%cluster_ctarank;" : "=r"(r));
  return r;
}
__device__ __forceinline__ uint32_t cluster_map_u32(uint32_t smem_addr, uint32_t rank) {
  uint32_t r;
  asm volatile("mapa.shared::cluster.u32 %0, %1, %2;" : "=r"(r) : "r"(smem_addr), "r"(rank));
  return r;
}
template <class T>
__device__ __forceinline__ T* cluster_map_ptr(T* p, uint32_t rank) {
  uint64_t r;
  asm volatile("mapa.u64 %0, %1, %2;" : "=l"(r) : "l"(reinterpret_cast<uint64_t>(p)), "r"(rank));
  return reinterpret_cast<T*>(r);
}
__device__ __forceinline__ void st_async_v4(uint32_t cluster_addr, uint32_t a, uint32_t b, uint32_t c, uint32_t d,
                                            uint32_t cluster_mbar) {
  asm volatile("st.async.weak.shared::cluster.mbarrier::complete_tx::bytes.v4.b32 [%0], {%1, %2, %3, %4}, [%5];"
               ::"r"(cluster_addr), "r"(a), "r"(b), "r"(c), "r"(d), "r"(cluster_mbar) : "memory");
}
__device__ __forceinline__ void st_async_b32(uint32_t cluster_addr, uint32_t v, uint32_t cluster_mbar) {
  asm volatile("st.async.weak.shared::cluster.mbarrier::complete_tx::bytes.b32 [%0], %1, [%2];"
               ::"r"(cluster_addr), "r"(v), "r"(cluster_mbar) : "memory");
}
__device__ __forceinline__ void cluster_sync_all() {
  asm volatile("barrier.cluster.arrive.release.aligned;\n\tbarrier.cluster.wait.acquire.aligned;" ::: "memory");
}

__device__ __forceinline__ uint64_t umma_desc_sw128(uint32_t smem_addr) {
  uint64_t d = 0;
  d |= (uint64_t)((smem_addr & 0x3FFFFu) >> 4);
  d |= (uint64_t)1 << 16;
  d |= (uint64_t)(1024 >> 4) << 32;
  d |= (uint64_t)1 << 46;
  d |= (uint64_t)2 << 61;
  return d;
}
__device__ __forceinline__ uint64_t umma_desc_k16_noswizzle(uint32_t smem_addr) {
  uint64_t d = 0;
  d |= (uint64_t)((smem_addr & 0x3FFFFu) >> 4);
  d |= (uint64_t)(128 >> 4) << 16;
  d |= (uint64_t)(256 >> 4) << 32;
  d |= (uint64_t)1 << 46;
  return d;
}
constexpr uint32_t kIdesc = (1u << 4) | (1u << 7) | (1u << 10) | ((128u >> 3) << 17) | ((128u >> 4) << 24);

__device__ __forceinline__ float softplus_fast(float x) {
  const float e = exp2f(fminf(x, 80.0f) * 1.4426950408889634f);
  return __log2f(1.0f + e) * 0.6931471805599453f;
}

__device__ __forceinline__ constexpr uint32_t umma_idesc_n(uint32_t n) {
  return (1u << 4) | (1u << 7) | (1u << 10) | ((n >> 3) << 17) | ((128u >> 4) << 24);
}

}
}
```

Measured before the change: 2870.

## Split pair variant by rows with M=64 MMAs instead of column exchange

The two-CTA pair variant now splits the 128-row tile into two 64-row halves, one per CTA. Each CTA runs M=64 UMMAs over all output columns using the 16x32bx2 TMEM load/store shapes. Previously the CTAs split output columns and swapped activations and score partials through cluster st.async with mbarriers. Removing that per-step cross-CTA exchange and its cluster synchronisation is meant to cut latency, at the cost of M=64 MMAs that use the tensor core less efficiently and issue more MMAs per layer. The pair path is also restricted to smaller L and constraint counts.

```diff
diff --git a/ethz-safe-learning_b200/csrc/rollout_tc.cu b/ethz-safe-learning_b200/csrc/rollout_tc.cu
--- a/ethz-safe-learning_b200/csrc/rollout_tc.cu
+++ b/ethz-safe-learning_b200/csrc/rollout_tc.cu
@@ -66,17 +66,15 @@
   }
 };
 
-struct AStorePair {
+struct AStoreTmem16 {
   uint32_t t_a;
-  uint32_t peer_slot;
-  uint32_t buf_off;
-  uint32_t peer_bar;
   __device__ __forceinline__ void store8(int k0, uint32_t p0, uint32_t p1, uint32_t p2, uint32_t p3) const {
     const uint32_t pk[4] = {p0, p1, p2, p3};
-    tmem_st<4>(t_a + (uint32_t)(k0 >> 1), pk);
-    st_async_v4(peer_slot + buf_off, p0, p1, p2, p3, peer_bar);
+    tmem_st16<4, 4>(t_a + (uint32_t)((k0 & ~15) >> 1), pk);
   }
 };
+template <>
+struct AStoreLanes16<AStoreTmem16> : std::true_type {};
 
 }
 
@@ -89,10 +87,12 @@
   constexpr int kTileWarps = Q * 4;
   constexpr int kEpiThreads = NTILES * kTileThreads;
   constexpr int kEpiWarps = kEpiThreads / 32;
-  constexpr int OW = (PAIR ? 32 : 64) / Q;
-  constexpr int NSL = PAIR ? 2 * Q : Q;
+  constexpr int kRows = PAIR ? 64 : 128;
+  constexpr int RQ = PAIR ? 2 * Q : Q;
+  constexpr int OW = 64 / RQ;
+  constexpr int NSL = RQ;
   constexpr int NB = OW / 8;
-  constexpr int HCOLS = 128 / Q;
+  constexpr int HCOLS = 128 / RQ;
   constexpr bool kDbl = NTILES == 1;
   static_assert(!kDbl || Q == 4, "the one-tile variants split the columns into halves of two column groups");
   constexpr int kTmemCols = 512;
@@ -101,6 +101,7 @@
   constexpr bool kPark = NTILES > 1;
   constexpr int kBarAcc = 2, kBarA = 2 + NTILES, kBarPart = 2 + 2 * NTILES, kBarFree = 2 + 3 * NTILES;
   constexpr int kBarAccHi = 6, kBarAHi = 7;
+  constexpr int kBarFreeHi = 8;
   extern __shared__ __align__(1024) uint8_t smem_raw[];
   const RowGeom& g = prm.g;
   const int L = prm.L;
@@ -110,9 +111,11 @@
   const uint32_t crank = PAIR ? cluster_ctarank() : 0u;
   const int n_items = (prm.n_tiles + NTILES - 1) / NTILES;
   const int cta_item0 = PAIR ? (int)(blockIdx.x >> 1) : (int)blockIdx.x;
+  const int row0 = (int)crank * kRows;
   const int n_ctas = PAIR ? (int)(gridDim.x >> 1) : (int)gridDim.x;
   const bool l0_pad_bias = tc_l0_pad_bias(O + A);
   constexpr int n_quarters = 4;
+  constexpr int n_lane_rows = kRows / 32;
   constexpr int tile_bar_threads = Q * 128 + 32;
   constexpr int half_bar_threads = Q * 64 + 32;
 
@@ -124,9 +127,7 @@
   float* pen_smem = scale_smem + 128;
   const int nparts = TRAJ ? 1 : 1 + prm.scorer.n_constraints;
   float* part_smem = pen_smem + kHeadParts * 64;
-  const int part_buf_floats = NTILES * NSL * nparts * 128;
-  uint4* xch_smem = reinterpret_cast<uint4*>(part_smem + (PAIR ? 2 : 1) * part_buf_floats);
-  uint4* noise_smem = xch_smem + (PAIR ? 2 * Q * 128 : 0);
+  uint4* noise_smem = reinterpret_cast<uint4*>(part_smem + NTILES * NSL * nparts * 128);
   uint32_t* rs_smem = reinterpret_cast<uint32_t*>(noise_smem + (kPark ? NB * kEpiThreads : 0));
   uint64_t* bars = reinterpret_cast<uint64_t*>(rs_smem + NTILES * 8 * 128);
   uint32_t* tmem_slot = reinterpret_cast<uint32_t*>(bars + 1 + NTILES + 2 + (kDbl ? 1 : 0));
@@ -148,7 +149,7 @@
   auto item_member = [&](int item) {
     int wm = -1;
     for (int q = 0; q < NTILES; ++q)
-      if (item * NTILES + q < prm.n_tiles && prm.tiles[item * NTILES + q].count > 0) wm = prm.tiles[item * NTILES + q].member;
+      if (item * NTILES + q < prm.n_tiles && prm.tiles[item * NTILES + q].count > row0) wm = prm.tiles[item * NTILES + q].member;
     return wm;
   };
   auto stage_weights = [&](int wm) {
@@ -172,10 +173,6 @@
       mbar_init(smem_u32(&bars[1 + j]), 1);
     }
     if (kDbl) mbar_init(smem_u32(&bars[3 + NTILES]), 1);
-    if (PAIR) {
-      mbar_init(smem_u32(&bars[1 + NTILES]), 1);
-      mbar_init(smem_u32(&bars[2 + NTILES]), 1);
-    }
     fence_barrier_init();
     w_state_sh[0] = -1;
     w_state_sh[1] = 0;
@@ -187,7 +184,7 @@
     if (ti < prm.n_tiles) {
       const Tile t = prm.tiles[ti];
       info.member = t.member; info.k0 = t.k0; info.count = t.count;
-      info.valid = t.count > 0 ? 1 : 0;
+      info.valid = t.count > row0 ? 1 : 0;
     }
     return info;
   };
@@ -208,15 +205,8 @@
                        l0_pad_bias ? O + A : -1, threadIdx.x, kEpiThreads);
     }
   }
-  if (PAIR && threadIdx.x == 0) {
-    const uint32_t per_step = crank == 0 ? (uint32_t)(kEpiThreads * 4 * nparts) : 0u;
-    mbar_expect_tx(smem_u32(&bars[2 + NTILES]), per_step + (uint32_t)(kEpiThreads * 16));
-    const uint32_t b0 = per_step + (1 < H ? (uint32_t)(kEpiThreads * 16) : 0u);
-    if (b0 != 0u) mbar_expect_tx(smem_u32(&bars[1 + NTILES]), b0);
-  }
   tc_fence_before();
   __syncthreads();
-  if (PAIR) cluster_sync_all();
   tc_fence_after();
   const uint32_t tmem_base = *tmem_slot;
   TLK(1);
@@ -264,7 +254,7 @@
         const uint32_t bar_lo = smem_u32(&bars[1]), bar_hi = smem_u32(&bars[3 + NTILES]);
         for (int t = 0; t < H; ++t) {
           for (int layer = 0; layer <= L; ++layer) {
-            mbar_wait(layer < L ? bar_lo : bar_hi, ph);
+            mbar_wait(PAIR || layer < L ? bar_lo : bar_hi, ph);
             tc_fence_before();
             named_bar_arrive_n(kBarAcc, half_bar_threads);
             mbar_wait(bar_hi, ph);
@@ -277,24 +267,14 @@
     } else if (warp >= kEpiWarps + NTILES) {
       const int j = warp - kEpiWarps - NTILES;
       const TileInfo tis = tinfo[j];
-      auto xbytes = [&](int t) -> uint32_t {
-        return (crank == 0 ? (uint32_t)(kEpiThreads * 4 * nparts) : 0u) + (t + 1 < H ? (uint32_t)(kEpiThreads * 16) : 0u);
-      };
-      const uint32_t xbar = smem_u32(&bars[1 + NTILES]);
-      if (PAIR && tis.valid && crank != 0 && late_gate(tis)) {
-        for (int ts = -1; ts + 1 < H; ++ts) {
-          mbar_wait(xbar + 8u * ((uint32_t)ts & 1u), (uint32_t)((ts + 1) >> 1) & 1u);
-          if (lane == 0 && xbytes(ts + 2) != 0u) mbar_expect_tx(xbar + 8u * ((uint32_t)ts & 1u), xbytes(ts + 2));
-        }
-      }
-      if (!TRAJ && tis.valid && crank == 0) {
+      if (!TRAJ && tis.valid) {
         const simba_scorer_t& sc = prm.scorer;
         const bool done_first = objective_done_first(prm.objective);
         uint32_t* my_rs = rs_smem + j * 8 * 128 + lane;
         const float* part_tile0 = part_smem + (j * NSL * nparts) * 128;
 #pragma unroll 1
-        for (int i = 0; i < n_quarters; ++i) {
-          const int row = lane + 32 * i;
+        for (int i = 0; i < n_lane_rows; ++i) {
+          const int row = row0 + lane + 32 * i;
 #pragma unroll
           for (int f = 0; f < 7; ++f) my_rs[f * 128 + 32 * i] = 0u;
           my_rs[7 * 128 + 32 * i] = row < tis.count ? (uint32_t)decode_row(g, tis.member, tis.k0 + row).out : 0xffffffffu;
@@ -302,17 +282,11 @@
         const bool live = late_gate(tis);
         for (int ts = -1; live && ts < H; ++ts) {
           named_bar_sync_n(kBarPart + j, tile_bar_threads);
-          const float* part_tile = part_tile0;
-          if (PAIR) {
-            mbar_wait(xbar + 8u * ((uint32_t)ts & 1u), (uint32_t)((ts + 1) >> 1) & 1u);
-            if (lane == 0 && ts + 2 < H) mbar_expect_tx(xbar + 8u * ((uint32_t)ts & 1u), xbytes(ts + 2));
-            part_tile += (ts & 1) * part_buf_floats;
-          }
 #pragma unroll 1
-          for (int i = 0; i < n_quarters; ++i) {
+          for (int i = 0; i < n_lane_rows; ++i) {
             uint32_t* q = my_rs + 32 * i;
             float nd, nc;
-            head_combine<NSL>(sc, part_tile + lane + 32 * i, nparts, nd, nc);
+            head_combine<NSL>(sc, part_tile0 + lane + 32 * i, nparts, nd, nc);
             if (ts < 0) {
               q[4 * 128] = __float_as_uint(nd);
               q[5 * 128] = __float_as_uint(nc);
@@ -334,11 +308,18 @@
               q[6 * 128] = rs.done ? 1u : 0u;
             }
           }
-          if (ts + 1 < H) named_bar_arrive_n(kBarFree + j, tile_bar_threads);
+          if (ts + 1 < H) {
+            if constexpr (PAIR) {
+              named_bar_arrive_n(kBarFree, half_bar_threads);
+              named_bar_arrive_n(kBarFreeHi, half_bar_threads);
+            } else {
+              named_bar_arrive_n(kBarFree + j, tile_bar_threads);
+            }
+          }
         }
         if (live && prm.row_return != nullptr) {
 #pragma unroll 1
-          for (int i = 0; i < n_quarters; ++i) {
+          for (int i = 0; i < n_lane_rows; ++i) {
             const uint32_t* q = my_rs + 32 * i;
             const uint32_t slot = q[7 * 128];
             if (slot != 0xffffffffu) {
@@ -363,7 +344,8 @@
         const bool live = late_gate(tinfo[j]);
         if constexpr (kDbl) {
           const uint32_t bar_acc_hi = smem_u32(&bars[3 + NTILES]);
-          constexpr uint32_t kIdesc64 = umma_idesc_n(64u), kIdesc32 = umma_idesc_n(32u);
+          constexpr uint32_t kM = PAIR ? 64u : 128u;
+          constexpr uint32_t kIdesc64 = umma_idesc_n(64u, kM), kIdesc32 = umma_idesc_n(32u, kM);
           uint32_t par = 0;
           auto mma4 = [&](uint32_t d, uint32_t a, uint64_t b, uint32_t idesc, int kb) {
 #pragma unroll
@@ -400,18 +382,21 @@
             }
             for (int layer = 1; layer <= L; ++layer) {
               const uint32_t d = d_tmem + par * 128, a = a_tmem + par * 64;
-              const bool own_head = PAIR && layer == L;
-              const uint32_t c0 = own_head ? crank * 32 : 0u, c1 = own_head ? 64u + crank * 32 : 64u;
-              const uint32_t idesc = own_head ? kIdesc32 : kIdesc64;
+              const bool pair_head = PAIR && layer == L;
+              const uint32_t c0 = 0u, c1 = pair_head ? 32u : 64u;
+              const uint32_t idesc = pair_head ? kIdesc32 : kIdesc64;
               const uint64_t bw = umma_desc_sw128(smem_u32(w_smem + kAtomBytes + (layer - 1) * 2 * kAtomBytes));
               const uint64_t b0 = bw + (uint64_t)((c0 * 128) >> 4), b1 = bw + (uint64_t)((c1 * 128) >> 4);
+              constexpr uint64_t kVarRows = (64 * 128) >> 4;
               const uint32_t bias_sm = smem_u32(biask_smem + layer * 4096);
               named_bar_sync_n(kBarA, half_bar_threads);
               tc_fence_after();
               TL(2 * layer);
               if (elect_one()) {
                 mma4(d + c0, a, b0, idesc, 0);
+                if (pair_head) mma4(d + c0 + 64, a, b0 + kVarRows, idesc, 0);
                 mma4(d + c1, a, b1, idesc, 0);
+                if (pair_head) mma4(d + c1 + 64, a, b1 + kVarRows, idesc, 0);
               }
               TL(2 * layer + 1);
               __syncwarp();
@@ -420,10 +405,14 @@
               TL(20 + 2 * layer);
               if (elect_one()) {
                 mma4(d + c0, a, b0, idesc, 4);
+                if (pair_head) mma4(d + c0 + 64, a, b0 + kVarRows, idesc, 4);
                 mma_bias(d + c0, bias_sm, c0, idesc);
+                if (pair_head) mma_bias(d + c0 + 64, bias_sm, c0 + 64, idesc);
                 umma_commit(bar_acc);
                 mma4(d + c1, a, b1, idesc, 4);
+                if (pair_head) mma4(d + c1 + 64, a, b1 + kVarRows, idesc, 4);
                 mma_bias(d + c1, bias_sm, c1, idesc);
+                if (pair_head) mma_bias(d + c1 + 64, bias_sm, c1 + 64, idesc);
                 umma_commit(bar_acc_hi);
               }
               TL(21 + 2 * layer);
@@ -469,11 +458,12 @@
       const int j = warp / kTileWarps;
       const int wl = warp - j * kTileWarps;
       const int cgp = wl >> 2;
-      const int r = (wl & 3) * 32 + lane;
+      const int r = PAIR ? (wl & 3) * 16 + (lane & 15) : (wl & 3) * 32 + lane;
+      const int sl = PAIR ? 2 * cgp + (lane >> 4) : cgp;
       const TileInfo ti = tinfo[j];
       if (ti.valid) {
-        const bool row_ok = r < ti.count;
-        const RowId id = decode_row(g, ti.member, ti.k0 + (row_ok ? r : 0));
+        const bool row_ok = row0 + r < ti.count;
+        const RowId id = decode_row(g, ti.member, ti.k0 + (row_ok ? row0 + r : 0));
         const uint32_t lane_base = tmem_base + ((uint32_t)((wl & 3) * 32) << 16);
         const uint32_t t_acc = lane_base + (uint32_t)j * 128;
         const uint32_t t_a = lane_base + (uint32_t)(kACol + j * 64);
@@ -483,40 +473,15 @@
         HeadCtx hc;
         hc.t_acc = t_acc;
         hc.t_state = lane_base + (uint32_t)(kStateCol + j * 64);
-        hc.o_base = (PAIR ? (int)crank * 32 : 0) + cgp * OW;
+        hc.o_base = sl * OW;
         hc.O = O; hc.A = A;
         hc.slice_bits = TRAJ ? 0u : head_slice_bits<OW>(sc, hc.o_base);
         hc.n_constraints = TRAJ ? 0 : sc.n_constraints;
         hc.scale_smem = scale_smem;
         hc.pen_smem = pen_smem;
-        float* part_slot0 = part_smem + ((j * NSL + (int)crank * Q + cgp) * nparts) * 128 + r;
-        hc.part = part_slot0 + (PAIR ? part_buf_floats : 0);
-        typename std::conditional<PAIR, AStorePair, AStoreTmem>::type astore;
+        hc.part = part_smem + ((j * NSL + sl) * nparts) * 128 + r;
+        typename std::conditional<PAIR, AStoreTmem16, AStoreTmem>::type astore;
         astore.t_a = t_a;
-        const uint32_t my_xbar = smem_u32(&bars[1 + NTILES]);
-        const uint32_t peer_xbar = PAIR ? cluster_map_u32(my_xbar, crank ^ 1u) : 0u;
-        const bool keeps_score = !TRAJ && (!PAIR || crank == 0);
-        const uint32_t part_remote0 = (PAIR && crank != 0) ? cluster_map_u32(smem_u32(part_slot0), 0u) : 0u;
-        if constexpr (PAIR) {
-          astore.peer_slot = cluster_map_u32(smem_u32(xch_smem + cgp * 128 + r), crank ^ 1u);
-          astore.buf_off = (uint32_t)(Q * 128 * sizeof(uint4));
-          astore.peer_bar = peer_xbar + 8u;
-          if (crank != 0) {
-            hc.part_remote = part_remote0 + (uint32_t)(part_buf_floats * sizeof(float));
-            hc.part_mbar = peer_xbar + 8u;
-          }
-        }
-        auto exchange = [&](int t, bool next_step) {
-          if constexpr (PAIR) {
-            const uint32_t b = (uint32_t)t & 1u;
-            if (next_step) {
-              mbar_wait(my_xbar + 8u * b, (uint32_t)((t + 1) >> 1) & 1u);
-              const uint4 v = xch_smem[(b * Q + cgp) * 128 + r];
-              const uint32_t pk[4] = {v.x, v.y, v.z, v.w};
-              tmem_st<4>(astore.t_a + (uint32_t)((((int)crank ^ 1) * 32 + cgp * 8) >> 1), pk);
-            }
-          }
-        };
         const float* s0_ptr = prm.states + (prm.state_per_row ? id.r_global : (int64_t)id.s) * prm.state_stride;
         typename std::conditional<FWD, ForwardSink, typename std::conditional<TRAJ, TrajSink, NoTraj>::type>::type sink{};
         if constexpr (FWD) {
@@ -545,8 +510,9 @@
         };
         auto gemm_par = [&](int t, int l) { return (uint32_t)(t * (L + 1) + l) & 1u; };
 
+        const int act_lo = PAIR ? (hc.o_base & ~15) : hc.o_base, act_w = PAIR ? 2 * OW : OW;
         const bool owns_actions = TRAJ ? (O < hc.o_base + OW) && (O + A > hc.o_base)
-                                       : (O >= hc.o_base) && (O < hc.o_base + OW);
+                                       : (O >= act_lo) && (O < act_lo + act_w);
         float act_pf[4] = {0.f, 0.f, 0.f, 0.f};
         auto prefetch_actions = [&](int tn) {
           if (owns_actions && row_ok && tn < H) {
@@ -604,10 +570,9 @@
         if constexpr (PAIR) head_first_pass_vals(hc, astore, s0v, act_pf);
         else head_first_pass<OW>(hc, astore, s0_ptr, row_ok, act_pf, sink);
         prefetch_actions(1);
-        exchange(-1, true);
         publish_a();
         TLK(3);
-        if (keeps_score) named_bar_arrive_n(kBarPart + j, tile_bar_threads);
+        if (!TRAJ) named_bar_arrive_n(kBarPart + j, tile_bar_threads);
 
         PhiloxState ps{0u, 0u, 0u, 0u, 0u, 0u};
         for (int t = 0; t < H; ++t) {
@@ -623,7 +588,14 @@
           for (int l = 0; l < L; ++l) {
             wait_accumulator();
             TL(1 + l * 4);
-            {
+            if constexpr (PAIR) {
+              uint32_t v[16], pk[8];
+              tmem_ld16<16, 16>(t_acc + gemm_par(t, l) * 128 + (uint32_t)(cgp * 32), v);
+              tmem_ld_wait();
+#pragma unroll
+              for (int q = 0; q < 8; ++q) pk[q] = pack_relu_bf16(__uint_as_float(v[2 * q]), __uint_as_float(v[2 * q + 1]));
+              tmem_st16<8, 8>(t_a + (gemm_par(t, l) ^ 1u) * 64 + (uint32_t)(cgp * 16), pk);
+            } else {
               constexpr int NLD = HCOLS / 32;
               uint32_t v[NLD][32];
 #pragma unroll
@@ -664,17 +636,11 @@
           }
 
           wait_accumulator();
-          if (keeps_score) named_bar_sync_n(kBarFree + j, tile_bar_threads);
+          if (!TRAJ) {
+            if constexpr (PAIR) named_bar_sync_n(cgp >= Q / 2 ? kBarFreeHi : kBarFree, half_bar_threads);
+            else named_bar_sync_n(kBarFree + j, tile_bar_threads);
+          }
           TL(40);
-          if constexpr (PAIR) {
-            hc.part = part_slot0 + (t & 1) * part_buf_floats;
-            astore.buf_off = (uint32_t)((t & 1) * Q * 128 * sizeof(uint4));
-            astore.peer_bar = peer_xbar + 8u * ((uint32_t)t & 1u);
-            if (crank != 0) {
-              hc.part_remote = part_remote0 + (uint32_t)((t & 1) * part_buf_floats * sizeof(float));
-              hc.part_mbar = astore.peer_bar;
-            }
-          }
           if constexpr (TRAJ && !FWD) {
             if (sink.row != nullptr) sink.row += O;
           }
@@ -686,9 +652,8 @@
           else if (prm.sampling_propagation) head_step_pass<OW, true>(hc, noise, astore, t + 1 < H, sink);
           else head_step_pass<OW, false>(hc, noise, astore, t + 1 < H, sink);
           TL(41);
-          exchange(t, t + 1 < H);
           if (t + 1 < H) publish_a();
-          if (keeps_score) named_bar_arrive_n(kBarPart + j, tile_bar_threads);
+          if (!TRAJ) named_bar_arrive_n(kBarPart + j, tile_bar_threads);
           TL(42);
         }
         TLK(6);
@@ -729,8 +694,7 @@
   size_t b = tc_member_bytes(L) + 4096;
   b += 128 * sizeof(float);
   b += kHeadParts * 64 * sizeof(float);
-  b += (size_t)ntiles * q * nparts * 128 * sizeof(float) * (pair ? 4 : 1);
-  if (pair) b += (size_t)2 * q * 128 * sizeof(uint4);
+  b += (size_t)ntiles * q * nparts * 128 * sizeof(float) * (pair ? 2 : 1);
   if (ntiles > 1)
     b += (size_t)(64 / q / 8) * (ntiles * q * 128) * sizeof(uint4);
   b += (size_t)8 * ntiles * 128 * sizeof(uint32_t);
@@ -790,7 +754,7 @@
 }
 
 bool rollout_tc_pair_fits(int L, int n_constraints) {
-  return tc_smem_bytes(L, 1, 4, 1 + n_constraints, true) + 1024 <= kMaxSmem;
+  return (L <= 3 || (L == 4 && n_constraints <= 3)) && tc_smem_bytes(L, 1, 4, 1 + n_constraints, true) + 1024 <= kMaxSmem;
 }
 
 template <int NTILES, int Q, bool PAIR, bool TRAJ, bool FWD = false>
diff --git a/ethz-safe-learning_b200/csrc/tc_head.cuh b/ethz-safe-learning_b200/csrc/tc_head.cuh
--- a/ethz-safe-learning_b200/csrc/tc_head.cuh
+++ b/ethz-safe-learning_b200/csrc/tc_head.cuh
@@ -1,4 +1,6 @@
 #pragma once
+#include <type_traits>
+
 #include "common.cuh"
 #include "tc_ptx.cuh"
 
@@ -104,8 +106,21 @@
   const float* scale_smem;
   const float* pen_smem;
   float* part;
-  uint32_t part_remote = 0, part_mbar = 0;
-};
+};
+
+template <class AStore>
+struct AStoreLanes16 : std::false_type {};
+
+template <bool kLanes16>
+__device__ __forceinline__ void head_ld8(uint32_t t_row, int col, uint32_t (&v)[8]) {
+  if constexpr (kLanes16) tmem_ld16<8, 8>(t_row + (uint32_t)(col & ~15), v);
+  else tmem_ld<8>(t_row + col, v);
+}
+template <bool kLanes16>
+__device__ __forceinline__ void head_st8(uint32_t t_row, int col, const uint32_t (&v)[8]) {
+  if constexpr (kLanes16) tmem_st16<8, 8>(t_row + (uint32_t)(col & ~15), v);
+  else tmem_st<8>(t_row + col, v);
+}
 
 __device__ __forceinline__ float head_stddev(float x_log2e) {
   float e, l, sd;
@@ -156,13 +171,6 @@
 }
 
 __device__ __forceinline__ void head_publish(const HeadCtx& c, float gmin, const float (&cmin)[SIMBA_MAX_CONSTRAINTS]) {
-  if (c.part_remote != 0u) {
-    st_async_b32(c.part_remote, __float_as_uint(gmin), c.part_mbar);
-#pragma unroll
-    for (int q = 0; q < SIMBA_MAX_CONSTRAINTS; ++q)
-      if (q < c.n_constraints) st_async_b32(c.part_remote + (uint32_t)((1 + q) * 128 * 4), __float_as_uint(cmin[q]), c.part_mbar);
-    return;
-  }
   c.part[0] = gmin;
 #pragma unroll
   for (int q = 0; q < SIMBA_MAX_CONSTRAINTS; ++q)
@@ -268,7 +276,7 @@
       if (oc + i == c.O + a) sv[i] = act0[a];
     st[i] = __float_as_uint(sv[i]);
   }
-  tmem_st<8>(c.t_state + oc, st);
+  head_st8<AStoreLanes16<AStore>::value>(c.t_state, oc, st);
   head_chunk_tail<64>(c, astore, oc, c.slice_bits & 31u, sv, true, gmin, cmin);
   head_publish(c, gmin, cmin);
 }
@@ -277,14 +285,16 @@
 __device__ __forceinline__ void head_step_pass(const HeadCtx& c, const Noise& noise, const AStore& astore,
                                                bool write_next, const Sink& sink = Sink()) {
   constexpr int NCH = OW / 8;
+  constexpr bool k16 = AStoreLanes16<AStore>::value;
+  static_assert(!k16 || NCH == 1, "the M = 64 layout gives a thread one 8-wide chunk");
   float gmin = INFINITY, cmin[SIMBA_MAX_CONSTRAINTS];
 #pragma unroll
   for (int q = 0; q < SIMBA_MAX_CONSTRAINTS; ++q) cmin[q] = INFINITY;
   static_assert(Sink::kState || kSample, "the forward form forms the variance");
   uint32_t vm[2][8], vv[2][8], st[2][8];
-  tmem_ld<8>(c.t_acc + c.o_base, vm[0]);
-  if (kSample) tmem_ld<8>(c.t_acc + kVar + c.o_base, vv[0]);
-  if constexpr (Sink::kState) tmem_ld<8>(c.t_state + c.o_base, st[0]);
+  head_ld8<k16>(c.t_acc, c.o_base, vm[0]);
+  if (kSample) head_ld8<k16>(c.t_acc + kVar, c.o_base, vv[0]);
+  if constexpr (Sink::kState) head_ld8<k16>(c.t_state, c.o_base, st[0]);
 #pragma unroll
   for (int ch = 0; ch < NCH; ++ch) {
     const int oc = c.o_base + ch * 8;
@@ -333,7 +343,7 @@
         uint32_t so[8];
 #pragma unroll
         for (int i = 0; i < 8; ++i) so[i] = __float_as_uint(sv[i]);
-        tmem_st<8>(c.t_state + oc, so);
+        head_st8<k16>(c.t_state, oc, so);
       }
       sink.put8(oc, sv);
       head_chunk_tail<kTW>(c, astore, oc, Sink::kScore ? (c.slice_bits >> (ch * 5)) & 31u : 0u, sv, write_next,
diff --git a/ethz-safe-learning_b200/csrc/tc_ptx.cuh b/ethz-safe-learning_b200/csrc/tc_ptx.cuh
--- a/ethz-safe-learning_b200/csrc/tc_ptx.cuh
+++ b/ethz-safe-learning_b200/csrc/tc_ptx.cuh
@@ -122,6 +122,28 @@
     asm volatile("tcgen05.st.sync.aligned.32x32b.x16.b32 [%0], {%1, %2, %3, %4, %5, %6, %7, %8, %9, %10, %11, %12, %13, %14, %15, %16};"
                  :: "r"(taddr), "r"(v[0]), "r"(v[1]), "r"(v[2]), "r"(v[3]), "r"(v[4]), "r"(v[5]), "r"(v[6]), "r"(v[7]), "r"(v[8]), "r"(v[9]), "r"(v[10]), "r"(v[11]), "r"(v[12]), "r"(v[13]), "r"(v[14]), "r"(v[15]) : "memory");
 }
+template <int N, int kSplit>
+__device__ __forceinline__ void tmem_ld16(uint32_t taddr, uint32_t (&v)[N]) {
+  static_assert(N == 8 || N == 16, "unsupported TMEM load width");
+  if constexpr (N == 8)
+    asm volatile("tcgen05.ld.sync.aligned.16x32bx2.x8.b32 {%0, %1, %2, %3, %4, %5, %6, %7}, [%8], %9;"
+                 : "=r"(v[0]), "=r"(v[1]), "=r"(v[2]), "=r"(v[3]), "=r"(v[4]), "=r"(v[5]), "=r"(v[6]), "=r"(v[7])
+                 : "r"(taddr), "n"(kSplit) : "memory");
+  if constexpr (N == 16)
+    asm volatile("tcgen05.ld.sync.aligned.16x32bx2.x16.b32 {%0, %1, %2, %3, %4, %5, %6, %7, %8, %9, %10, %11, %12, %13, %14, %15}, [%16], %17;"
+                 : "=r"(v[0]), "=r"(v[1]), "=r"(v[2]), "=r"(v[3]), "=r"(v[4]), "=r"(v[5]), "=r"(v[6]), "=r"(v[7]), "=r"(v[8]), "=r"(v[9]), "=r"(v[10]), "=r"(v[11]), "=r"(v[12]), "=r"(v[13]), "=r"(v[14]), "=r"(v[15])
+                 : "r"(taddr), "n"(kSplit) : "memory");
+}
+template <int N, int kSplit>
+__device__ __forceinline__ void tmem_st16(uint32_t taddr, const uint32_t (&v)[N]) {
+  static_assert(N == 4 || N == 8, "unsupported TMEM store width");
+  if constexpr (N == 4)
+    asm volatile("tcgen05.st.sync.aligned.16x32bx2.x4.b32 [%0], %1, {%2, %3, %4, %5};"
+                 :: "r"(taddr), "n"(kSplit), "r"(v[0]), "r"(v[1]), "r"(v[2]), "r"(v[3]) : "memory");
+  if constexpr (N == 8)
+    asm volatile("tcgen05.st.sync.aligned.16x32bx2.x8.b32 [%0], %1, {%2, %3, %4, %5, %6, %7, %8, %9};"
+                 :: "r"(taddr), "n"(kSplit), "r"(v[0]), "r"(v[1]), "r"(v[2]), "r"(v[3]), "r"(v[4]), "r"(v[5]), "r"(v[6]), "r"(v[7]) : "memory");
+}
 __device__ __forceinline__ void tmem_ld_wait() {
   asm volatile("tcgen05.wait::ld.sync.aligned;" ::: "memory");
 }
@@ -216,29 +238,6 @@
   uint32_t r;
   asm volatile("mov.u32 %0, %%cluster_ctarank;" : "=r"(r));
   return r;
-}
-__device__ __forceinline__ uint32_t cluster_map_u32(uint32_t smem_addr, uint32_t rank) {
-  uint32_t r;
-  asm volatile("mapa.shared::cluster.u32 %0, %1, %2;" : "=r"(r) : "r"(smem_addr), "r"(rank));
-  return r;
-}
-template <class T>
-__device__ __forceinline__ T* cluster_map_ptr(T* p, uint32_t rank) {
-  uint64_t r;
-  asm volatile("mapa.u64 %0, %1, %2;" : "=l"(r) : "l"(reinterpret_cast<uint64_t>(p)), "r"(rank));
-  return reinterpret_cast<T*>(r);
-}
-__device__ __forceinline__ void st_async_v4(uint32_t cluster_addr, uint32_t a, uint32_t b, uint32_t c, uint32_t d,
-                                            uint32_t cluster_mbar) {
-  asm volatile("st.async.weak.shared::cluster.mbarrier::complete_tx::bytes.v4.b32 [%0], {%1, %2, %3, %4}, [%5];"
-               ::"r"(cluster_addr), "r"(a), "r"(b), "r"(c), "r"(d), "r"(cluster_mbar) : "memory");
-}
-__device__ __forceinline__ void st_async_b32(uint32_t cluster_addr, uint32_t v, uint32_t cluster_mbar) {
-  asm volatile("st.async.weak.shared::cluster.mbarrier::complete_tx::bytes.b32 [%0], %1, [%2];"
-               ::"r"(cluster_addr), "r"(v), "r"(cluster_mbar) : "memory");
-}
-__device__ __forceinline__ void cluster_sync_all() {
-  asm volatile("barrier.cluster.arrive.release.aligned;\n\tbarrier.cluster.wait.acquire.aligned;" ::: "memory");
 }
 
 __device__ __forceinline__ uint64_t umma_desc_sw128(uint32_t smem_addr) {
@@ -265,9 +264,9 @@
   return __log2f(1.0f + e) * 0.6931471805599453f;
 }
 
-__device__ __forceinline__ constexpr uint32_t umma_idesc_n(uint32_t n) {
-  return (1u << 4) | (1u << 7) | (1u << 10) | ((n >> 3) << 17) | ((128u >> 4) << 24);
-}
-
-}
-}
+__device__ __forceinline__ constexpr uint32_t umma_idesc_n(uint32_t n, uint32_t m = 128u) {
+  return (1u << 4) | (1u << 7) | (1u << 10) | ((n >> 3) << 17) | ((m >> 4) << 24);
+}
+
+}
+}
```

After: 3185 (median of 6 runs). 11.0% higher.
